# VincentGourbin/ltx-video-swift-mlx

Measured on NVIDIA B200. Metric: dit_steps_per_s, higher is better.
Workload: dtype bf16

## Files before the change

include/ltxcuda.h:

```cpp
#ifndef LTXCUDA_H_
#define LTXCUDA_H_

#include <stddef.h>
#include <stdint.h>

#ifdef __cplusplus
extern "C" {
#endif
#if defined(__GNUC__)
#pragma GCC visibility push(default)
#endif

#define LTX_OK 0
#define LTX_ERR_INVALID_CONFIGURATION 1
#define LTX_ERR_INVALID_ARGUMENT 2
#define LTX_ERR_CUDA 3
#define LTX_ERR_WEIGHTS 4
#define LTX_ERR_UNSUPPORTED 5

typedef enum { LTX_F32 = 0, LTX_BF16 = 1, LTX_F16 = 2 } ltx_dtype;

typedef struct ltx_ctx ltx_ctx;

typedef struct {
  int32_t num_layers;
  int32_t num_heads;
  int32_t head_dim;
  int32_t in_channels;
  int32_t out_channels;
  int32_t caption_channels;
  int32_t ffn_mult;
  float rope_theta;
  int32_t max_pos[3];
  float timestep_scale_multiplier;
  float norm_eps;
  int32_t vae_latent_channels;
  int32_t vae_base_channels;
  int32_t vae_blocks_per_stage;
  int32_t vae_patch_size;
  int32_t vae_encoder_base_channels;
  int32_t upscaler_mid_channels;
  int32_t upscaler_blocks;
  int32_t audio_num_heads;
  int32_t audio_head_dim;
  int32_t audio_in_channels;
  int32_t audio_max_pos;
} ltx_config;

void ltx_config_default(ltx_config* cfg);
const char* ltx_version(void);

int ltx_ctx_create(const ltx_config* cfg, int device, ltx_ctx** out);
int ltx_ctx_destroy(ltx_ctx* ctx);
const char* ltx_last_error(const ltx_ctx* ctx);
int ltx_sync(ltx_ctx* ctx);

int ltx_load_tensor(ltx_ctx* ctx, const char* key, const void* host_data, ltx_dtype dtype, const int64_t* shape, int ndim);
int ltx_load_safetensors(ltx_ctx* ctx, const char* path, int which, int* n_loaded);
int ltx_map_weight_key(int which, const char* file_key, char* out, size_t cap);
int ltx_fuse_lora(ltx_ctx* ctx, const char* key, const void* down, const void* up, ltx_dtype dtype, int rank, float scale);
int ltx_set_precision(ltx_ctx* ctx, int bits);
int ltx_set_quant_storage(ltx_ctx* ctx, int materialise);
int ltx_init_random_weights(ltx_ctx* ctx, int which, uint64_t seed);
int ltx_finalize_weights(ltx_ctx* ctx, int quant_bits, int group_size);

#define LTX_MAX_FLAG_BLOCKS 64
typedef struct {
  int32_t n_stg_blocks;
  int32_t stg_blocks[LTX_MAX_FLAG_BLOCKS];
  int32_t skip_self_attn;
  int32_t skip_ff;
  int32_t n_cas_blocks;
  int32_t cas_blocks[LTX_MAX_FLAG_BLOCKS];
  float cross_attn_scale;
  uint64_t context_key;
} ltx_dit_flags;

int ltx_dit_forward(ltx_ctx* ctx, const void* latent, ltx_dtype latent_dtype, const void* context, ltx_dtype context_dtype,
                    const float* timesteps, int ts_per_token, const int32_t* mask, int B, int N, int S, int F, int H,
                    int W, const ltx_dit_flags* flags, float* out_velocity);
int ltx_dit_forward_dev(ltx_ctx* ctx, const void* latent, ltx_dtype latent_dtype, const void* context,
                        ltx_dtype context_dtype, const float* timesteps, int ts_per_token, const int32_t* mask, int B, int N,
                        int S, int F, int H, int W, const ltx_dit_flags* flags, float* out_velocity);
int ltx_av_forward(ltx_ctx* ctx, const void* video_latent, ltx_dtype video_dtype, const void* audio_latent, ltx_dtype audio_dtype,
                   const void* video_context, const void* audio_context, ltx_dtype context_dtype, float video_sigma,
                   float audio_sigma, const int32_t* video_mask, const int32_t* audio_mask, int N, int Ta, int S, int F, int H,
                   int W, uint64_t context_key, float* out_video, float* out_audio);
int ltx_av_forward_dev(ltx_ctx* ctx, const void* video_latent, ltx_dtype video_dtype, const void* audio_latent,
                       ltx_dtype audio_dtype, const void* video_context, const void* audio_context, ltx_dtype context_dtype,
                       const float* video_sigma, const float* audio_sigma, const int32_t* video_mask, const int32_t* audio_mask,
                       int N, int Ta, int S, int F, int H, int W, uint64_t context_key, float* out_video, float* out_audio);
int ltx_av_forward_tokens(ltx_ctx* ctx, const void* video_latent, ltx_dtype video_dtype, const void* audio_latent,
                          ltx_dtype audio_dtype, const void* video_context, const void* audio_context, ltx_dtype context_dtype,
                          const float* video_sigmas, float audio_sigma, const int32_t* video_mask, const int32_t* audio_mask, int N,
                          int Ta, int S, int F, int H, int W, uint64_t context_key, float* out_video, float* out_audio);
int ltx_av_forward_tokens_dev(ltx_ctx* ctx, const void* video_latent, ltx_dtype video_dtype, const void* audio_latent,
                              ltx_dtype audio_dtype, const void* video_context, const void* audio_context, ltx_dtype context_dtype,
                              const float* video_sigmas, const float* audio_sigma, const int32_t* video_mask,
                              const int32_t* audio_mask, int N, int Ta, int S, int F, int H, int W, uint64_t context_key,
                              float* out_video, float* out_audio);
int ltx_av_forward_batch(ltx_ctx* ctx, const void* video_latent, ltx_dtype video_dtype, const void* audio_latent,
                         ltx_dtype audio_dtype, const void* video_context, const void* audio_context, ltx_dtype context_dtype,
                         const float* video_sigmas, int video_ts_per_token, const float* audio_sigmas, const int32_t* video_mask,
                         const int32_t* audio_mask, int B, int N, int Ta, int S, int F, int H, int W, uint64_t context_key,
                         float* out_video, float* out_audio);
int ltx_av_forward_batch_dev(ltx_ctx* ctx, const void* video_latent, ltx_dtype video_dtype, const void* audio_latent,
                             ltx_dtype audio_dtype, const void* video_context, const void* audio_context, ltx_dtype context_dtype,
                             const float* video_sigmas, int video_ts_per_token, const float* audio_sigmas,
                             const int32_t* video_mask, const int32_t* audio_mask, int B, int N, int Ta, int S, int F, int H, int W,
                             uint64_t context_key, float* out_video, float* out_audio);
int ltx_dit_clear_caches(ltx_ctx* ctx);

int ltx_guided_euler_step(ltx_ctx* ctx, float* latent, const float* v_cond, const float* v_uncond, const float* v_stg,
                          float* v_prev, int use_prev, size_t n, float cfg_scale, float rescale_phi, float stg_scale,
                          float ge_gamma, float sigma, float sigma_next);
int ltx_guided_euler_step_dev(ltx_ctx* ctx, float* latent, const float* v_cond, const float* v_uncond, const float* v_stg,
                              float* v_prev, int use_prev, size_t n, float cfg_scale, float rescale_phi, float stg_scale,
                              float ge_gamma, float sigma, float sigma_next);

typedef struct {
  float sigma, sigma_next;
  float cfg_scale;
  float rescale_phi;
  float stg_scale;
  float ge_gamma;
  int32_t n_stg_blocks;
  int32_t stg_blocks[LTX_MAX_FLAG_BLOCKS];
  int32_t step_index;
  int32_t i2v_frame0_conditioned;
  int32_t disable_stg_prefix_sharing;
  int32_t disable_batched_cfg;
} ltx_step_params;
int ltx_denoise_begin(ltx_ctx* ctx, const float* noise, int F, int H, int W, float sigma0, const void* context,
                      ltx_dtype context_dtype, const int32_t* mask, const void* neg_context, const int32_t* neg_mask, int S);
int ltx_denoise_step(ltx_ctx* ctx, const ltx_step_params* p);
int ltx_denoise_get_latent(ltx_ctx* ctx, float* latent_out);
int ltx_denoise_latent_dev(ltx_ctx* ctx, float** latent_dev);

int ltx_av_denoise_begin(ltx_ctx* ctx, const float* video_noise, const float* audio_noise, int F, int H, int W, int Ta,
                         float sigma0, const void* video_context, const void* audio_context, ltx_dtype context_dtype,
                         const int32_t* mask, const void* neg_video_context, const void* neg_audio_context,
                         const int32_t* neg_mask, int S);
int ltx_av_denoise_step(ltx_ctx* ctx, const ltx_step_params* p);
int ltx_av_denoise_get_latents(ltx_ctx* ctx, float* video_latent_out, float* audio_latent_out);

int ltx_vae_decode(ltx_ctx* ctx, const float* latent, int Fp, int Hp, int Wp, float timestep, const float* decode_noise,
                   int causal, float* out_frames);
int ltx_vae_decode_dev(ltx_ctx* ctx, const float* latent, int Fp, int Hp, int Wp, float timestep,
                       const float* decode_noise, int causal, float* out_frames);
int ltx_vae_tiled_frames(int Fp, int tile_size, int tile_overlap);
int ltx_vae_decode_tiled(ltx_ctx* ctx, const float* latent, int Fp, int Hp, int Wp, float timestep, const float* decode_noise,
                         int causal, int tile_size, int tile_overlap, float* out_frames, int* out_num_frames);
int ltx_vae_decode_tiled_dev(ltx_ctx* ctx, const float* latent, int Fp, int Hp, int Wp, float timestep,
                             const float* decode_noise, int causal, int tile_size, int tile_overlap, float* out_frames,
                             int* out_num_frames);

int ltx_vae_encode(ltx_ctx* ctx, const float* pixels, int T, int H, int W, int normalize, float* latent_out);
int ltx_vae_encode_dev(ltx_ctx* ctx, const float* pixels, int T, int H, int W, int normalize, float* latent_out);

int ltx_upscale_latent(ltx_ctx* ctx, const float* latent, int F, int H, int W, float* out);
int ltx_upscale_latent_dev(ltx_ctx* ctx, const float* latent, int F, int H, int W, float* out);

int ltx_adain_filter(ltx_ctx* ctx, float* latent, size_t n_per_channel, const float* reference, size_t n_ref_per_channel,
                     int channels, float factor);
int ltx_adain_filter_dev(ltx_ctx* ctx, float* latent, size_t n_per_channel, const float* reference, size_t n_ref_per_channel,
                         int channels, float factor);

int ltx_denoise_begin_from_latent(ltx_ctx* ctx, const float* latent, const float* noise, float noise_scale,
                                  const float* frame0_latent, int F, int H, int W, const void* context, ltx_dtype context_dtype,
                                  const int32_t* mask, const void* neg_context, const int32_t* neg_mask, int S);
int ltx_denoise_upscale_stage(ltx_ctx* ctx, const float* noise, float noise_scale, float adain_factor);
int ltx_denoise_set_frame0(ltx_ctx* ctx, const float* frame0_latent);

int ltx_dist_get_unique_id(void* id_out_128);
int ltx_dist_init(ltx_ctx* ctx, const void* unique_id_128, int rank, int world_size, int sp_size, int pass_groups);
int ltx_dist_info(const ltx_ctx* ctx, int* rank, int* world_size, int* sp_size, int* pass_groups);
int ltx_dist_p2p_active(const ltx_ctx* ctx);
int ltx_dist_init_local(ltx_ctx** contexts, int n, int sp_size, int pass_groups);
int ltx_dist_shutdown(ltx_ctx* ctx);

int ltx_host_alloc(void** ptr, size_t bytes);
int ltx_host_free(void* ptr);

uint64_t ltx_launch_count(const ltx_ctx* ctx);
int ltx_get_stream(ltx_ctx* ctx, void** stream);
int ltx_set_profiling(ltx_ctx* ctx, int enabled);
int ltx_set_graphs(ltx_ctx* ctx, int enabled);
int ltx_graph_stats(const ltx_ctx* ctx, uint64_t* captures, uint64_t* replays);
int ltx_get_profile(ltx_ctx* ctx, double* ms, double* flops, double* bytes, uint64_t* counts, int n_classes);

int ltx_op_gemm(ltx_ctx* ctx, const void* A, const void* B, const float* bias, void* C, int M, int N, int K, int mode,
                int force_bn);
int ltx_op_gemm_blocked(ltx_ctx* ctx, const void* A, const void* B, const float* bias, void* plain_out, void* blocks_out, int M, int N,
                        int K, int col_from, int col_block, int64_t block_stride, int force_bn);
int ltx_op_gemm_resid(ltx_ctx* ctx, const void* A, const void* B, const float* bias, float* x, const float* gate_a,
                      const float* gate_b, void* shadow, int M, int N, int K, float scale);
int ltx_op_gemm_skinny(ltx_ctx* ctx, const void* A, const void* B, const float* bias, void* out, float* x, const float* gate_a,
                       const float* gate_b, int rows_per_gate, int M, int N, int K, int mode, int items, int64_t vt_item_ld);
int ltx_op_quantize(ltx_ctx* ctx, const void* w_bf16, int N, int K, int bits, void* q_out, float* scales_out, float* biases_out);
int ltx_op_dequantize(ltx_ctx* ctx, const void* q, const float* scales, const float* biases, int N, int K, int bits, void* w_bf16);
int ltx_op_gemm_q(ltx_ctx* ctx, const void* A, const void* q, const float* scales, const float* biases, int bits,
                  const float* bias, void* C, int M, int N, int K, int mode, int force_bn);
int ltx_op_quantize_fp8(ltx_ctx* ctx, const void* x_bf16, int M, int K, int64_t ld, void* codes, float* scales);
int ltx_op_gemm_fp8(ltx_ctx* ctx, const void* Aq, const float* sa, const void* Bq, const float* sb, const float* bias, void* C, int M,
                    int N, int K, int mode, int force_bn);
int ltx_op_gemm_fp8_ex(ltx_ctx* ctx, const void* Aq, const float* sa, const void* Bq, const float* sb, const float* bias, void* C,
                       void* Ct, int tsplit_col, int64_t ldt, float* x, const float* gate_a, const float* gate_b, void* shadow,
                       int M, int N, int K, int force_bn);
int ltx_op_attention(ltx_ctx* ctx, const void* Q, const void* K, const void* Vt, int64_t ldvb, const float* key_bias, void* O,
                     int B, int H, int Nq, int Nk, float scale);
int ltx_op_attention_hd(ltx_ctx* ctx, const void* Q, const void* K, const void* Vt, int64_t ldvb, const float* key_bias, void* O,
                        int B, int H, int head_dim, int Nq, int Nk, float scale);
int ltx_op_attention_blocks(ltx_ctx* ctx, const void* Q, const void* K, const void* Vt, int64_t ldvb, int H, int Nq, int Nk,
                            float scale, void* const* o_blocks, int n_blocks, int rows_per_block);
int ltx_op_rmsnorm_mod(ltx_ctx* ctx, const float* x, void* out_bf16, int M, int D, const float* tbl_shift,
                       const float* tbl_scale, const float* ada_shift, const float* ada_scale, float eps, int layernorm);
int ltx_op_qknorm_rope(ltx_ctx* ctx, void* x_bf16, int M, int D, const float* w, const float* cos_tab, const float* sin_tab,
                       int rows_per_rope, float eps);
int ltx_conv3d_plan(int T, int H, int W, int Cin, int Cout, int mode, int ntaps, int sm_count, int32_t* plan7);
int ltx_op_conv3d(ltx_ctx* ctx, const float* x, const void* w_bf16_27_O_I, const float* bias, float* out, int T, int H,
                  int W, int Cin, int Cout, int causal);
int ltx_op_vae_prep(ltx_ctx* ctx, const float* x, void* out_pad_bf16, int T, int H, int W, int C, int mode, const float* a,
                    const float* b, int pad);
int ltx_op_vae_halo_fill(ltx_ctx* ctx, void* vol_bf16, int T, int H, int W, int C, int pad);
int ltx_op_conv3d_epi(ltx_ctx* ctx, const void* x_pad_bf16, const void* w_bf16, const float* bias, int T, int H, int W, int Cin,
                      int Cout, int ntaps, int mode, float* out, const float* resid, int t_shift, int no_clip, void* next_pad_bf16,
                      const float* next_scale, const float* next_shift, int next_tshift);

#if defined(__GNUC__)
#pragma GCC visibility pop
#endif
#ifdef __cplusplus
}
#endif
#endif
```

ltx-video-swift-mlx_b200/_lib.py:

```python
from __future__ import annotations

import ctypes as C
import os

_HERE = os.path.dirname(os.path.abspath(__file__))
LIB_PATH = os.path.join(_HERE, "libltxcuda.so")

LTX_F32, LTX_BF16, LTX_F16 = 0, 1, 2
LTX_MAX_FLAG_BLOCKS = 64


class LtxConfig(C.Structure):
    _fields_ = [
        ("num_layers", C.c_int32), ("num_heads", C.c_int32), ("head_dim", C.c_int32), ("in_channels", C.c_int32),
        ("out_channels", C.c_int32), ("caption_channels", C.c_int32), ("ffn_mult", C.c_int32), ("rope_theta", C.c_float),
        ("max_pos", C.c_int32 * 3), ("timestep_scale_multiplier", C.c_float), ("norm_eps", C.c_float),
        ("vae_latent_channels", C.c_int32), ("vae_base_channels", C.c_int32), ("vae_blocks_per_stage", C.c_int32),
        ("vae_patch_size", C.c_int32), ("vae_encoder_base_channels", C.c_int32), ("upscaler_mid_channels", C.c_int32),
        ("upscaler_blocks", C.c_int32), ("audio_num_heads", C.c_int32), ("audio_head_dim", C.c_int32),
        ("audio_in_channels", C.c_int32), ("audio_max_pos", C.c_int32),
    ]


class LtxDitFlags(C.Structure):
    _fields_ = [
        ("n_stg_blocks", C.c_int32), ("stg_blocks", C.c_int32 * LTX_MAX_FLAG_BLOCKS), ("skip_self_attn", C.c_int32),
        ("skip_ff", C.c_int32), ("n_cas_blocks", C.c_int32), ("cas_blocks", C.c_int32 * LTX_MAX_FLAG_BLOCKS),
        ("cross_attn_scale", C.c_float), ("context_key", C.c_uint64),
    ]


class LtxStepParams(C.Structure):
    _fields_ = [
        ("sigma", C.c_float), ("sigma_next", C.c_float), ("cfg_scale", C.c_float), ("rescale_phi", C.c_float),
        ("stg_scale", C.c_float), ("ge_gamma", C.c_float), ("n_stg_blocks", C.c_int32),
        ("stg_blocks", C.c_int32 * LTX_MAX_FLAG_BLOCKS), ("step_index", C.c_int32),
        ("i2v_frame0_conditioned", C.c_int32), ("disable_stg_prefix_sharing", C.c_int32), ("disable_batched_cfg", C.c_int32),
    ]


_P, _I, _F, _U64, _SZ, _I64 = C.c_void_p, C.c_int, C.c_float, C.c_uint64, C.c_size_t, C.c_int64
SIGNATURES = {
    "ltx_config_default": (None, [C.POINTER(LtxConfig)]),
    "ltx_version": (C.c_char_p, []),
    "ltx_ctx_create": (_I, [C.POINTER(LtxConfig), _I, C.POINTER(_P)]),
    "ltx_ctx_destroy": (_I, [_P]),
    "ltx_last_error": (C.c_char_p, [_P]),
    "ltx_sync": (_I, [_P]),
    "ltx_load_tensor": (_I, [_P, C.c_char_p, _P, _I, C.POINTER(_I64), _I]),
    "ltx_load_safetensors": (_I, [_P, C.c_char_p, _I, C.POINTER(_I)]),
    "ltx_map_weight_key": (_I, [_I, C.c_char_p, C.c_char_p, _SZ]),
    "ltx_fuse_lora": (_I, [_P, C.c_char_p, _P, _P, _I, _I, _F]),
    "ltx_set_precision": (_I, [_P, _I]),
    "ltx_set_quant_storage": (_I, [_P, _I]),
    "ltx_init_random_weights": (_I, [_P, _I, _U64]),
    "ltx_finalize_weights": (_I, [_P, _I, _I]),
    "ltx_dit_forward": (_I, [_P, _P, _I, _P, _I, _P, _I, _P, _I, _I, _I, _I, _I, _I, C.POINTER(LtxDitFlags), _P]),
    "ltx_dit_forward_dev": (_I, [_P, _P, _I, _P, _I, _P, _I, _P, _I, _I, _I, _I, _I, _I, C.POINTER(LtxDitFlags), _P]),
    "ltx_av_forward": (_I, [_P, _P, _I, _P, _I, _P, _P, _I, _F, _F, _P, _P, _I, _I, _I, _I, _I, _I, _U64, _P, _P]),
    "ltx_av_forward_dev": (_I, [_P, _P, _I, _P, _I, _P, _P, _I, _P, _P, _P, _P, _I, _I, _I, _I, _I, _I, _U64, _P, _P]),
    "ltx_av_forward_tokens": (_I, [_P, _P, _I, _P, _I, _P, _P, _I, _P, _F, _P, _P, _I, _I, _I, _I, _I, _I, _U64, _P, _P]),
    "ltx_av_forward_tokens_dev": (_I, [_P, _P, _I, _P, _I, _P, _P, _I, _P, _P, _P, _P, _I, _I, _I, _I, _I, _I, _U64, _P, _P]),
    "ltx_av_forward_batch": (_I, [_P, _P, _I, _P, _I, _P, _P, _I, _P, _I, _P, _P, _P, _I, _I, _I, _I, _I, _I, _I, _U64, _P, _P]),
    "ltx_av_forward_batch_dev": (_I, [_P, _P, _I, _P, _I, _P, _P, _I, _P, _I, _P, _P, _P, _I, _I, _I, _I, _I, _I, _I, _U64, _P, _P]),
    "ltx_dit_clear_caches": (_I, [_P]),
    "ltx_guided_euler_step": (_I, [_P, _P, _P, _P, _P, _P, _I, _SZ, _F, _F, _F, _F, _F, _F]),
    "ltx_guided_euler_step_dev": (_I, [_P, _P, _P, _P, _P, _P, _I, _SZ, _F, _F, _F, _F, _F, _F]),
    "ltx_denoise_begin": (_I, [_P, _P, _I, _I, _I, _F, _P, _I, _P, _P, _P, _I]),
    "ltx_denoise_step": (_I, [_P, C.POINTER(LtxStepParams)]),
    "ltx_denoise_get_latent": (_I, [_P, _P]),
    "ltx_denoise_latent_dev": (_I, [_P, C.POINTER(_P)]),
    "ltx_av_denoise_begin": (_I, [_P, _P, _P, _I, _I, _I, _I, _F, _P, _P, _I, _P, _P, _P, _P, _I]),
    "ltx_av_denoise_step": (_I, [_P, C.POINTER(LtxStepParams)]),
    "ltx_av_denoise_get_latents": (_I, [_P, _P, _P]),
    "ltx_vae_decode": (_I, [_P, _P, _I, _I, _I, _F, _P, _I, _P]),
    "ltx_vae_decode_dev": (_I, [_P, _P, _I, _I, _I, _F, _P, _I, _P]),
    "ltx_vae_tiled_frames": (_I, [_I, _I, _I]),
    "ltx_vae_decode_tiled": (_I, [_P, _P, _I, _I, _I, _F, _P, _I, _I, _I, _P, _P]),
    "ltx_vae_decode_tiled_dev": (_I, [_P, _P, _I, _I, _I, _F, _P, _I, _I, _I, _P, _P]),
    "ltx_vae_encode": (_I, [_P, _P, _I, _I, _I, _I, _P]),
    "ltx_vae_encode_dev": (_I, [_P, _P, _I, _I, _I, _I, _P]),
    "ltx_upscale_latent": (_I, [_P, _P, _I, _I, _I, _P]),
    "ltx_upscale_latent_dev": (_I, [_P, _P, _I, _I, _I, _P]),
    "ltx_adain_filter": (_I, [_P, _P, _SZ, _P, _SZ, _I, _F]),
    "ltx_adain_filter_dev": (_I, [_P, _P, _SZ, _P, _SZ, _I, _F]),
    "ltx_denoise_begin_from_latent": (_I, [_P, _P, _P, _F, _P, _I, _I, _I, _P, _I, _P, _P, _P, _I]),
    "ltx_denoise_upscale_stage": (_I, [_P, _P, _F, _F]),
    "ltx_denoise_set_frame0": (_I, [_P, _P]),
    "ltx_dist_get_unique_id": (_I, [_P]),
    "ltx_dist_init": (_I, [_P, _P, _I, _I, _I, _I]),
    "ltx_dist_init_local": (_I, [_P, _I, _I, _I]),
    "ltx_dist_shutdown": (_I, [_P]),
    "ltx_dist_p2p_active": (_I, [_P]),
    "ltx_dist_info": (_I, [_P, C.POINTER(_I), C.POINTER(_I), C.POINTER(_I), C.POINTER(_I)]),
    "ltx_host_alloc": (_I, [C.POINTER(_P), _SZ]),
    "ltx_host_free": (_I, [_P]),
    "ltx_launch_count": (_U64, [_P]),
    "ltx_get_stream": (_I, [_P, C.POINTER(_P)]),
    "ltx_set_profiling": (_I, [_P, _I]),
    "ltx_set_graphs": (_I, [_P, _I]),
    "ltx_graph_stats": (_I, [_P, _P, _P]),
    "ltx_get_profile": (_I, [_P, _P, _P, _P, _P, _I]),
    "ltx_op_gemm": (_I, [_P, _P, _P, _P, _P, _I, _I, _I, _I, _I]),
    "ltx_op_gemm_blocked": (_I, [_P, _P, _P, _P, _P, _P, _I, _I, _I, _I, _I, C.c_int64, _I]),
    "ltx_op_gemm_resid": (_I, [_P, _P, _P, _P, _P, _P, _P, _P, _I, _I, _I, _F]),
    "ltx_op_gemm_skinny": (_I, [_P, _P, _P, _P, _P, _P, _P, _P, _I, _I, _I, _I, _I, _I, C.c_int64]),
    "ltx_op_quantize": (_I, [_P, _P, _I, _I, _I, _P, _P, _P]),
    "ltx_op_dequantize": (_I, [_P, _P, _P, _P, _I, _I, _I, _P]),
    "ltx_op_gemm_q": (_I, [_P, _P, _P, _P, _P, _I, _P, _P, _I, _I, _I, _I, _I]),
    "ltx_op_quantize_fp8": (_I, [_P, _P, _I, _I, _I64, _P, _P]),
    "ltx_op_gemm_fp8": (_I, [_P, _P, _P, _P, _P, _P, _P, _I, _I, _I, _I, _I]),
    "ltx_op_gemm_fp8_ex": (_I, [_P, _P, _P, _P, _P, _P, _P, _P, _I, _I64, _P, _P, _P, _P, _I, _I, _I, _I]),
    "ltx_op_attention": (_I, [_P, _P, _P, _P, _I64, _P, _P, _I, _I, _I, _I, _F]),
    "ltx_op_attention_hd": (_I, [_P, _P, _P, _P, _I64, _P, _P, _I, _I, _I, _I, _I, _F]),
    "ltx_op_attention_blocks": (_I, [_P, _P, _P, _P, _I64, _I, _I, _I, _F, C.POINTER(_P), _I, _I]),
    "ltx_op_rmsnorm_mod": (_I, [_P, _P, _P, _I, _I, _P, _P, _P, _P, _F, _I]),
    "ltx_op_qknorm_rope": (_I, [_P, _P, _I, _I, _P, _P, _P, _I, _F]),
    "ltx_op_conv3d": (_I, [_P, _P, _P, _P, _P, _I, _I, _I, _I, _I, _I]),
    "ltx_conv3d_plan": (_I, [_I, _I, _I, _I, _I, _I, _I, _I, C.POINTER(C.c_int32)]),
    "ltx_op_vae_prep": (_I, [_P, _P, _P, _I, _I, _I, _I, _I, _P, _P, _I]),
    "ltx_op_vae_halo_fill": (_I, [_P, _P, _I, _I, _I, _I, _I]),
    "ltx_op_conv3d_epi": (_I, [_P, _P, _P, _P, _I, _I, _I, _I, _I, _I, _I, _P, _P, _I, _I, _P, _P, _P, _I]),
}

_lib = None


def load() -> C.CDLL:
    global _lib
    if _lib is not None:
        return _lib
    if not os.path.exists(LIB_PATH):
        raise RuntimeError(
            f"{LIB_PATH} is missing: build it with `bash ltx-video-swift-mlx_b200/csrc/build.sh` "
            "(there is no CPU / PyTorch fallback for the product path)")
    lib = C.CDLL(LIB_PATH)
    for name, (res, args) in SIGNATURES.items():
        fn = getattr(lib, name)
        fn.restype = res
        fn.argtypes = args
    _lib = lib
    return lib


class LtxError(RuntimeError):

    def __init__(self, code: int, message: str):
        super().__init__(f"[ltxcuda error {code}] {message}")
        self.code = code
```

ltx-video-swift-mlx_b200/csrc/api.cu:

```cuda
#include <cstring>

#include "ctx.h"

using namespace ltx;

namespace {

thread_local std::string g_create_error;

template <typename Fn>
int guarded(ltx_ctx* c, Fn&& fn) {
  if (!c) return LTX_ERR_INVALID_ARGUMENT;
  try {
    LTX_CUDA(cudaSetDevice(c->device));
    fn();
    return LTX_OK;
  } catch (const LtxError& e) {
    c->last_error = e.what();
    return e.code;
  } catch (const std::exception& e) {
    c->last_error = e.what();
    return LTX_ERR_CUDA;
  }
}
// ... 915 lines not shown
    h2d(c, c->s_latent, video_noise, n * 4);
    h2d(c, c->s_alat, audio_noise, na * 4);
    {
      ProfScope ps(c, PROF_OTHER, 0.0, 8.0 * (n + na), 2);
      launch_scale_f32(c->s_latent.as<float>(), sigma0, static_cast<int64_t>(n), c->stream);
      launch_scale_f32(c->s_alat.as<float>(), sigma0, static_cast<int64_t>(na), c->stream);
    }
    const size_t cbytes = static_cast<size_t>(S) * g.caption_channels * dsize(context_dtype);
    h2d(c, c->s_ctx_pos, video_context, cbytes);
    h2d(c, c->s_actx_pos, audio_context, cbytes);
    c->s_has_mask_pos = mask != nullptr;
    if (mask) h2d(c, c->s_mask_pos, mask, static_cast<size_t>(S) * 4);
    c->s_has_neg = neg_video_context != nullptr;
    if (c->s_has_neg) {
      h2d(c, c->s_ctx_neg, neg_video_context, cbytes);
      h2d(c, c->s_actx_neg, neg_audio_context, cbytes);
      c->s_has_mask_neg = neg_mask != nullptr;
      if (neg_mask) h2d(c, c->s_mask_neg, neg_mask, static_cast<size_t>(S) * 4);
      c->s_ctx_pair.reserve(2 * cbytes);
      c->s_actx_pair.reserve(2 * cbytes);
      LTX_CUDA(cudaMemcpyAsync(c->s_ctx_pair.ptr, c->s_ctx_pos.ptr, cbytes, cudaMemcpyDeviceToDevice, c->stream));
      LTX_CUDA(cudaMemcpyAsync(c->s_ctx_pair.as<uint8_t>() + cbytes, c->s_ctx_neg.ptr, cbytes, cudaMemcpyDeviceToDevice, c->stream));
      LTX_CUDA(cudaMemcpyAsync(c->s_actx_pair.ptr, c->s_actx_pos.ptr, cbytes, cudaMemcpyDeviceToDevice, c->stream));
      LTX_CUDA(cudaMemcpyAsync(c->s_actx_pair.as<uint8_t>() + cbytes, c->s_actx_neg.ptr, cbytes, cudaMemcpyDeviceToDevice, c->stream));
      if (mask || neg_mask) {
        std::vector<int32_t> pm(static_cast<size_t>(2) * S, 1);
        if (mask) memcpy(pm.data(), mask, static_cast<size_t>(S) * 4);
        if (neg_mask) memcpy(pm.data() + S, neg_mask, static_cast<size_t>(S) * 4);
        h2d(c, c->s_mask_pair, pm.data(), pm.size() * 4);
        LTX_CUDA(cudaStreamSynchronize(c->stream));
      }
      c->s_tok.reserve(2 * n * 2);
      c->vel.reserve(2 * n * 4);
      c->s_alat_pair.reserve(2 * na * 4);
    }
    c->s_avc.reserve((c->s_has_neg ? 2 : 1) * na * 4);
    c->s_avu.reserve(na * 4);
    c->scratch.reserve(64 * sizeof(double));
    c->s_serial += 2;
    dit_clear_caches(c);
    LTX_CUDA(cudaStreamSynchronize(c->stream));
  });
}

int ltx_av_denoise_step(ltx_ctx* c, const ltx_step_params* p) {
  return guarded(c, [&] {
    av_precision_check(c);
    LTX_CHECK(p != nullptr && c->s_F > 0 && c->s_Ta > 0, LTX_ERR_INVALID_ARGUMENT, "av_denoise_step before av_denoise_begin");
    LTX_CHECK(p->sigma > 0.f, LTX_ERR_INVALID_ARGUMENT, "sigma must be > 0");
    LTX_CHECK(p->stg_scale == 0.f && p->ge_gamma == 0.f, LTX_ERR_UNSUPPORTED,
              "the audio + video loop has no STG / GE terms (Pipeline/LTXPipeline.swift:1300-1404)");
    const ltx_config& g = c->cfg;
    const int C = g.in_channels, F = c->s_F, H = c->s_H, W = c->s_W, S = c->s_S, Ta = c->s_Ta;
    const int T = F * H * W;
    const size_t n = static_cast<size_t>(C) * T, na = static_cast<size_t>(Ta) * c->av.Cin;
    cudaStream_t st = c->stream;
    {
      ProfScope ps(c, PROF_OTHER, 0.0, 6.0 * n);
      launch_patchify(c->s_latent.as<float>(), c->s_tok.as<bf16>(), nullptr, C, T, st);
    }
    const bool use_cfg = p->cfg_scale > 1.0f && c->s_has_neg;
    const bool batched = batched_cfg_env() && use_cfg && c->dist.groups == 1 && !(c->dist.comm_world && c->dist.sp > 1) &&
                         !p->disable_batched_cfg;
    const int nb = batched ? 2 : 1;
    const float sig2[2] = {p->sigma, p->sigma};
    LTX_CUDA(cudaMemcpyAsync(c->s_sigma.ptr, sig2, 8, cudaMemcpyHostToDevice, st));
    const bool i2v = p->i2v_frame0_conditioned != 0;
    const float* ts_dev = c->s_sigma.as<float>();
    if (i2v) {
      c->s_ts.reserve(static_cast<size_t>(nb) * T * 4);
      ProfScope ps(c, PROF_OTHER, 0.0, 4.0 * nb * T);
      launch_fill_token_timesteps(c->s_ts.as<float>(), nb * T, T, H * W, c->s_sigma.as<float>(), st);
      ts_dev = c->s_ts.as<float>();
    }
    const uint64_t key_pos = 0x6000000000000000ull + c->s_serial, key_neg = key_pos + 1;
    const uint64_t key_pair = 0x6800000000000000ull + c->s_serial;
    auto pass = [&](bool neg, float* v_lat, float* a_vel) {
      const int32_t* mk = neg ? (c->s_has_mask_neg ? c->s_mask_neg.as<int32_t>() : nullptr)
                              : (c->s_has_mask_pos ? c->s_mask_pos.as<int32_t>() : nullptr);
      dit_av_forward_dev(c, c->s_tok.ptr, LTX_BF16, c->s_alat.ptr, LTX_F32, neg ? c->s_ctx_neg.ptr : c->s_ctx_pos.ptr,
                         neg ? c->s_actx_neg.ptr : c->s_actx_pos.ptr, c->s_ctx_dtype, ts_dev, i2v ? 1 : 0, c->s_sigma.as<float>(), mk,
                         mk, 1, T, Ta, S, F, H, W, neg ? key_neg : key_pos, c->vel.as<float>(), a_vel);
      ProfScope ps(c, PROF_OTHER, 0.0, 8.0 * n);
      launch_unpatchify(c->vel.as<float>(), v_lat, C, T, st);
    };
    float* avu = c->s_avu.as<float>();
    if (batched) {
      bf16* tok = c->s_tok.as<bf16>();
      float* alat2 = c->s_alat_pair.as<float>();
      LTX_CUDA(cudaMemcpyAsync(tok + n, tok, n * 2, cudaMemcpyDeviceToDevice, st));
      LTX_CUDA(cudaMemcpyAsync(alat2, c->s_alat.ptr, na * 4, cudaMemcpyDeviceToDevice, st));
      LTX_CUDA(cudaMemcpyAsync(alat2 + na, c->s_alat.ptr, na * 4, cudaMemcpyDeviceToDevice, st));
      const int32_t* mk = (c->s_has_mask_pos || c->s_has_mask_neg) ? c->s_mask_pair.as<int32_t>() : nullptr;
      avu = c->s_avc.as<float>() + na;
      dit_av_forward_dev(c, tok, LTX_BF16, alat2, LTX_F32, c->s_ctx_pair.ptr, c->s_actx_pair.ptr, c->s_ctx_dtype, ts_dev, i2v ? 1 : 0,
                         c->s_sigma.as<float>(), mk, mk, 2, T, Ta, S, F, H, W, key_pair, c->vel.as<float>(), c->s_avc.as<float>());
      ProfScope ps(c, PROF_OTHER, 0.0, 16.0 * n, 2);
      launch_unpatchify(c->vel.as<float>(), c->s_vc.as<float>(), C, T, st);
      launch_unpatchify(c->vel.as<float>() + n, c->s_vu.as<float>(), C, T, st);
    } else {
      pass(false, c->s_vc.as<float>(), c->s_avc.as<float>());
      if (use_cfg) pass(true, c->s_vu.as<float>(), avu);
    }
    GuidedEulerArgs a;
    a.latent = c->s_latent.as<float>(); a.v_cond = c->s_vc.as<float>();
    a.v_uncond = use_cfg ? c->s_vu.as<float>() : nullptr;
    a.v_stg = nullptr; a.v_prev = nullptr; a.use_prev = 0;
    a.v_out = nullptr; a.n = n; a.cfg = use_cfg ? p->cfg_scale : 1.0f; a.phi = use_cfg ? p->rescale_phi : 0.0f; a.stg = 0.f;
    a.ge_gamma = 0.f; a.sigma = p->sigma; a.sigma_next = p->sigma_next; a.scratch = c->scratch.as<double>();
    if (i2v) { a.period = static_cast<size_t>(T); a.frozen = static_cast<size_t>(H) * W; }
    ProfScope ps(c, PROF_OTHER, 0.0, 4.0 * n * (3.0 + (use_cfg ? 1.0 : 0.0)) + 4.0 * na * (3.0 + (use_cfg ? 1.0 : 0.0)),
                 ((use_cfg && p->rescale_phi > 0.f) ? 2 : 1) + 1);
    launch_guided_euler(a, st);
    const float dt = static_cast<float>(static_cast<double>(p->sigma_next) - static_cast<double>(p->sigma));
    launch_audio_cfg_euler(c->s_alat.as<float>(), c->s_avc.as<float>(), use_cfg ? avu : nullptr, p->cfg_scale, dt,
                           static_cast<int64_t>(na), st);
  });
}

int ltx_av_denoise_get_latents(ltx_ctx* c, float* video_out, float* audio_out) {
  return guarded(c, [&] {
    LTX_CHECK(c->s_F > 0 && c->s_Ta > 0, LTX_ERR_INVALID_ARGUMENT, "no audio + video denoise session");
    const size_t n = static_cast<size_t>(c->cfg.in_channels) * c->s_F * c->s_H * c->s_W;
    if (video_out) LTX_CUDA(cudaMemcpyAsync(video_out, c->s_latent.ptr, n * 4, cudaMemcpyDeviceToHost, c->stream));
    if (audio_out)
      LTX_CUDA(cudaMemcpyAsync(audio_out, c->s_alat.ptr, static_cast<size_t>(c->s_Ta) * c->av.Cin * 4, cudaMemcpyDeviceToHost,
                               c->stream));
    LTX_CUDA(cudaStreamSynchronize(c->stream));
  });
}

int ltx_vae_decode_dev(ltx_ctx* c, const float* latent, int Fp, int Hp, int Wp, float timestep, const float* decode_noise,
                       int causal, float* out_frames) {
  return guarded(c, [&] { vae_decode_dev(c, latent, Fp, Hp, Wp, timestep, decode_noise, causal, out_frames); });
}

int ltx_vae_decode(ltx_ctx* c, const float* latent, int Fp, int Hp, int Wp, float timestep, const float* decode_noise,
                   int causal, float* out_frames) {
  return guarded(c, [&] {
    LTX_CHECK(latent && out_frames && Fp > 0 && Hp > 0 && Wp > 0, LTX_ERR_INVALID_ARGUMENT, "bad vae_decode arguments");
    const size_t n = static_cast<size_t>(c->cfg.vae_latent_channels) * Fp * Hp * Wp;
    h2d(c, c->v_lat, latent, n * 4);
    const float* nz = nullptr;
    if (timestep >= 0.f) {
      LTX_CHECK(decode_noise != nullptr, LTX_ERR_INVALID_ARGUMENT, "decode_noise is required when timestep >= 0");
      h2d(c, c->v_noise, decode_noise, n * 4);
      nz = c->v_noise.as<float>();
    }
    const size_t fo = static_cast<size_t>(8 * (Fp - 1) + 1) * (32 * Hp) * (32 * Wp) * 3;
    c->v_frames.reserve(fo * 4);
    vae_decode_dev(c, c->v_lat.as<float>(), Fp, Hp, Wp, timestep, nz, causal, c->v_frames.as<float>());
    LTX_CUDA(cudaMemcpyAsync(out_frames, c->v_frames.ptr, fo * 4, cudaMemcpyDeviceToHost, c->stream));
    LTX_CUDA(cudaStreamSynchronize(c->stream));
  });
}

int ltx_vae_tiled_frames(int Fp, int tile_size, int tile_overlap) {
  if (Fp <= 0 || (tile_size > 0 && Fp > tile_size && (tile_overlap < 0 || tile_overlap >= tile_size))) return -1;
  return vae_tiled_frames(Fp, tile_size, tile_overlap);
}

int ltx_vae_decode_tiled_dev(ltx_ctx* c, const float* latent, int Fp, int Hp, int Wp, float timestep, const float* decode_noise,
                             int causal, int tile_size, int tile_overlap, float* out_frames, int* out_num_frames) {
  return guarded(c, [&] {
    const int n = vae_decode_tiled_dev(c, latent, Fp, Hp, Wp, timestep, decode_noise, causal, tile_size, tile_overlap, out_frames);
    if (out_num_frames) *out_num_frames = n;
  });
}

int ltx_vae_decode_tiled(ltx_ctx* c, const float* latent, int Fp, int Hp, int Wp, float timestep, const float* decode_noise,
                         int causal, int tile_size, int tile_overlap, float* out_frames, int* out_num_frames) {
  return guarded(c, [&] {
    LTX_CHECK(latent && out_frames && Fp > 0 && Hp > 0 && Wp > 0, LTX_ERR_INVALID_ARGUMENT, "bad vae_decode arguments");
    const int nf = ltx_vae_tiled_frames(Fp, tile_size, tile_overlap);
    LTX_CHECK(nf > 0, LTX_ERR_INVALID_ARGUMENT, "temporal tile overlap must be in [0, tile size)");
    const size_t n = static_cast<size_t>(c->cfg.vae_latent_channels) * Fp * Hp * Wp;
    h2d(c, c->v_lat, latent, n * 4);
    const float* nz = nullptr;
    if (timestep >= 0.f) {
      LTX_CHECK(decode_noise != nullptr, LTX_ERR_INVALID_ARGUMENT, "decode_noise is required when timestep >= 0");
      h2d(c, c->v_noise, decode_noise, n * 4);
      nz = c->v_noise.as<float>();
    }
    const size_t fe = static_cast<size_t>(32 * Hp) * (32 * Wp) * 3;
    c->v_frames.reserve(static_cast<size_t>(nf) * fe * 4);
    const int got = vae_decode_tiled_dev(c, c->v_lat.as<float>(), Fp, Hp, Wp, timestep, nz, causal, tile_size, tile_overlap,
                                         c->v_frames.as<float>());
    LTX_CHECK(got == nf, LTX_ERR_CUDA, "tiled decode frame count mismatch");
    if (out_num_frames) *out_num_frames = got;
    LTX_CUDA(cudaMemcpyAsync(out_frames, c->v_frames.ptr, static_cast<size_t>(got) * fe * 4, cudaMemcpyDeviceToHost, c->stream));
    LTX_CUDA(cudaStreamSynchronize(c->stream));
  });
}

int ltx_vae_encode_dev(ltx_ctx* c, const float* pixels, int T, int H, int W, int normalize, float* latent_out) {
  return guarded(c, [&] { vae_encode_dev(c, pixels, T, H, W, normalize, latent_out); });
}

int ltx_vae_encode(ltx_ctx* c, const float* pixels, int T, int H, int W, int normalize, float* latent_out) {
  return guarded(c, [&] {
    LTX_CHECK(pixels && latent_out && T >= 1 && H >= 64 && W >= 64 && H % 32 == 0 && W % 32 == 0, LTX_ERR_INVALID_ARGUMENT,
              "bad vae_encode arguments");
    const size_t n_in = static_cast<size_t>(3) * T * H * W;
    const size_t n_out = static_cast<size_t>(c->cfg.vae_latent_channels) * ((T + 7) / 8) * (H / 32) * (W / 32);
    h2d(c, c->u_in, pixels, n_in * 4);
    c->u_out.reserve(n_out * 4);
    vae_encode_dev(c, c->u_in.as<float>(), T, H, W, normalize, c->u_out.as<float>());
    LTX_CUDA(cudaMemcpyAsync(latent_out, c->u_out.ptr, n_out * 4, cudaMemcpyDeviceToHost, c->stream));
    LTX_CUDA(cudaStreamSynchronize(c->stream));
  });
}

int ltx_upscale_latent_dev(ltx_ctx* c, const float* latent, int F, int H, int W, float* out) {
  return guarded(c, [&] { upscale_latent_dev(c, latent, F, H, W, out); });
}

int ltx_upscale_latent(ltx_ctx* c, const float* latent, int F, int H, int W, float* out) {
  return guarded(c, [&] {
    LTX_CHECK(latent && out && F >= 1 && H > 1 && W > 1, LTX_ERR_INVALID_ARGUMENT, "bad upscale_latent arguments");
    const size_t n = static_cast<size_t>(c->cfg.vae_latent_channels) * F * H * W;
    h2d(c, c->u_in, latent, n * 4);
    c->u_out.reserve(4 * n * 4);
    upscale_latent_dev(c, c->u_in.as<float>(), F, H, W, c->u_out.as<float>());
    LTX_CUDA(cudaMemcpyAsync(out, c->u_out.ptr, 4 * n * 4, cudaMemcpyDeviceToHost, c->stream));
    LTX_CUDA(cudaStreamSynchronize(c->stream));
  });
}

int ltx_adain_filter_dev(ltx_ctx* c, float* latent, size_t n_per_channel, const float* reference, size_t n_ref_per_channel,
                         int channels, float factor) {
  return guarded(c, [&] {
    adain_filter_dev(c, latent, static_cast<int64_t>(n_per_channel), reference, static_cast<int64_t>(n_ref_per_channel), channels,
                     factor);
  });
}

int ltx_adain_filter(ltx_ctx* c, float* latent, size_t n_per_channel, const float* reference, size_t n_ref_per_channel, int channels,
                     float factor) {
  return guarded(c, [&] {
    LTX_CHECK(latent && reference && channels > 0, LTX_ERR_INVALID_ARGUMENT, "bad adain arguments");
    h2d(c, c->u_in, latent, n_per_channel * channels * 4);
    h2d(c, c->u_ref, reference, n_ref_per_channel * channels * 4);
    adain_filter_dev(c, c->u_in.as<float>(), static_cast<int64_t>(n_per_channel), c->u_ref.as<float>(),
                     static_cast<int64_t>(n_ref_per_channel), channels, factor);
    LTX_CUDA(cudaMemcpyAsync(latent, c->u_in.ptr, n_per_channel * channels * 4, cudaMemcpyDeviceToHost, c->stream));
    LTX_CUDA(cudaStreamSynchronize(c->stream));
  });
}

int ltx_op_gemm(ltx_ctx* c, const void* A, const void* B, const float* bias, void* C, int M, int N, int K, int mode,
                int force_bn) {
  return guarded(c, [&] {
    GemmEpi e;
    e.mode = mode; e.out = C; e.ldo = N; e.bias = bias;
    LTX_CHECK(mode == EPI_BF16 || mode == EPI_GELU_BF16 || mode == EPI_F32 || mode == EPI_SILU_BF16, LTX_ERR_INVALID_ARGUMENT, "bad mode");
    if (force_bn == -1) {
      LTX_CHECK(gemm_skinny_eligible(K, K, M, N, K, e, 0), LTX_ERR_INVALID_ARGUMENT, "shape not eligible for the skinny GEMM");
      launch_gemm_skinny(reinterpret_cast<const bf16*>(A), K, reinterpret_cast<const bf16*>(B), K, M, N, K, e, c->stream);
    } else if (force_bn == -2 || force_bn == -3) {
      LTX_CHECK(gemm_swapab_eligible(K, K, M, N, K, e), LTX_ERR_INVALID_ARGUMENT, "shape not eligible for the swap-AB GEMM");
      if (force_bn == -2) gemm_attach_workspace(c, e);
      launch_gemm_swapab(reinterpret_cast<const bf16*>(A), K, reinterpret_cast<const bf16*>(B), K, M, N, K, e, c->stream);
    } else {
      launch_gemm(reinterpret_cast<const bf16*>(A), K, reinterpret_cast<const bf16*>(B), K, M, N, K, e, c->stream, force_bn);
    }
    c->launches++;
  });
}

int ltx_op_gemm_blocked(ltx_ctx* c, const void* A, const void* B, const float* bias, void* plain_out, void* blocks_out, int M, int N,
                        int K, int col_from, int col_block, int64_t block_stride, int force_bn) {
  return guarded(c, [&] {
    LTX_CHECK(col_block > 0 && col_from >= 0 && col_from < N && (N - col_from) % col_block == 0 && (N - col_from) / col_block <= LTX_MAX_PEERS,
              LTX_ERR_INVALID_ARGUMENT, "bad column blocking");
    GemmEpi e;
    e.mode = EPI_BF16; e.out = plain_out; e.ldo = col_from > 0 ? col_from : col_block; e.bias = bias;
    e.col_block = col_block; e.col_block_from = col_from; e.blocked_ld = col_block; e.use_col_ptrs = 1;
    for (int j = 0; j < (N - col_from) / col_block; ++j)
      e.col_ptrs.p[j] = reinterpret_cast<bf16*>(blocks_out) + static_cast<int64_t>(j) * block_stride;
    if (force_bn == -2) {
      gemm_attach_workspace(c, e);
      launch_gemm_swapab(reinterpret_cast<const bf16*>(A), K, reinterpret_cast<const bf16*>(B), K, M, N, K, e, c->stream);
    } else {
      launch_gemm(reinterpret_cast<const bf16*>(A), K, reinterpret_cast<const bf16*>(B), K, M, N, K, e, c->stream, force_bn);
    }
    c->launches++;
  });
}

int ltx_op_gemm_resid(ltx_ctx* c, const void* A, const void* B, const float* bias, float* x, const float* gate_a,
                      const float* gate_b, void* shadow, int M, int N, int K, float scale) {
  return guarded(c, [&] {
    GemmEpi e;
    e.mode = EPI_GATE_RESID; e.resid = x; e.ldr = N; e.bias = bias; e.gate_a = gate_a; e.gate_b = gate_b; e.gate_ld = 0;
    e.rows_per_gate = M > 0 ? M : 1; e.shadow = reinterpret_cast<bf16*>(shadow); e.lds = N; e.scale = scale;
    if (M > 32 && M <= 512) gemm_attach_workspace(c, e);
    const char* fb = getenv("LTX_GEMM_FORCE_BN");
    launch_gemm(reinterpret_cast<const bf16*>(A), K, reinterpret_cast<const bf16*>(B), K, M, N, K, e, c->stream, fb ? atoi(fb) : 0, 0, 0,
                32 );
    c->launches++;
  });
}

int ltx_op_gemm_skinny(ltx_ctx* c, const void* A, const void* B, const float* bias, void* out, float* x, const float* gate_a,
                       const float* gate_b, int rows_per_gate, int M, int N, int K, int mode, int items, int64_t vt_item_ld) {
  return guarded(c, [&] {
    LTX_CHECK(A && B && (mode == EPI_GATE_RESID ? x != nullptr : out != nullptr) && (items == 1 || items == 2) &&
                  (vt_item_ld == 0 || (M % items == 0 && vt_item_ld >= M / items)),
              LTX_ERR_INVALID_ARGUMENT, "bad skinny GEMM arguments");
    LTX_CHECK(mode >= EPI_BF16 && mode <= EPI_SILU_BF16 && (vt_item_ld == 0 || mode == EPI_BF16), LTX_ERR_INVALID_ARGUMENT, "bad mode");
    GemmEpi e;
    e.mode = mode; e.bias = bias;
    if (mode == EPI_GATE_RESID) {
      e.resid = x; e.ldr = N; e.gate_a = gate_a; e.gate_b = gate_b; e.gate_ld = N;
      e.rows_per_gate = rows_per_gate > 0 ? rows_per_gate : M;
    } else if (vt_item_ld > 0) {
      e.out = out; e.ldo = items * vt_item_ld; e.transpose_out = 1;
      if (items > 1) { e.t_item_rows = M / items; e.t_item_ld = vt_item_ld; }
    } else {
      e.out = out; e.ldo = N;
    }
    LTX_CHECK(gemm_skinny_eligible(K, K, M, N, K, e, 0, 32 * items), LTX_ERR_INVALID_ARGUMENT, "shape not eligible for the skinny GEMM");
    launch_gemm(reinterpret_cast<const bf16*>(A), K, reinterpret_cast<const bf16*>(B), K, M, N, K, e, c->stream, 0, 0, 0, 32 * items);
    c->launches++;
  });
}

int ltx_op_quantize(ltx_ctx* c, const void* w_bf16, int N, int K, int bits, void* q_out, float* scales_out, float* biases_out) {
  return guarded(c, [&] {
    launch_quantize(reinterpret_cast<const bf16*>(w_bf16), N, K, bits, reinterpret_cast<uint8_t*>(q_out), scales_out, biases_out,
                    c->stream);
    c->launches++;
  });
}

int ltx_op_dequantize(ltx_ctx* c, const void* q, const float* scales, const float* biases, int N, int K, int bits, void* w_bf16) {
  return guarded(c, [&] {
    QuantW W;
    W.q = reinterpret_cast<const uint8_t*>(q); W.scales = scales; W.biases = biases; W.bits = bits; W.n = N; W.k = K;
    launch_dequantize(W, reinterpret_cast<bf16*>(w_bf16), c->stream);
    c->launches++;
  });
}

int ltx_op_gemm_q(ltx_ctx* c, const void* A, const void* q, const float* scales, const float* biases, int bits, const float* bias,
                  void* C, int M, int N, int K, int mode, int force_bn) {
  return guarded(c, [&] {
    LTX_CHECK(mode == EPI_BF16 || mode == EPI_GELU_BF16 || mode == EPI_F32, LTX_ERR_INVALID_ARGUMENT, "bad mode");
    QuantW W;
    W.q = reinterpret_cast<const uint8_t*>(q); W.scales = scales; W.biases = biases; W.bits = bits; W.n = N; W.k = K;
    GemmEpi e;
    e.mode = mode; e.out = C; e.ldo = N; e.bias = bias;
    launch_gemm_q(reinterpret_cast<const bf16*>(A), K, W, M, N, K, e, c->stream, force_bn);
    c->launches++;
  });
}

int ltx_op_quantize_fp8(ltx_ctx* c, const void* x_bf16, int M, int K, int64_t ld, void* codes, float* scales) {
  return guarded(c, [&] {
    LTX_CHECK(x_bf16 && codes && scales, LTX_ERR_INVALID_ARGUMENT, "null tensor");
    launch_quantize_rows_fp8(reinterpret_cast<const bf16*>(x_bf16), ld, M, K, reinterpret_cast<uint8_t*>(codes), scales, c->stream);
    c->launches++;
  });
}

int ltx_op_gemm_fp8(ltx_ctx* c, const void* Aq, const float* sa, const void* Bq, const float* sb, const float* bias, void* C, int M,
                    int N, int K, int mode, int force_bn) {
  return guarded(c, [&] {
    LTX_CHECK(Aq && sa && Bq && sb && C, LTX_ERR_INVALID_ARGUMENT, "null tensor");
    LTX_CHECK(mode == EPI_BF16 || mode == EPI_GELU_BF16 || mode == EPI_F32 || mode == EPI_SILU_BF16, LTX_ERR_INVALID_ARGUMENT, "bad mode");
    GemmEpi e;
    e.mode = mode; e.out = C; e.ldo = N; e.bias = bias;
    launch_gemm_fp8(reinterpret_cast<const uint8_t*>(Aq), K, sa, reinterpret_cast<const uint8_t*>(Bq), K, sb, M, N, K, e, c->stream,
                    force_bn);
    c->launches++;
  });
}

int ltx_op_gemm_fp8_ex(ltx_ctx* c, const void* Aq, const float* sa, const void* Bq, const float* sb, const float* bias, void* C,
                       void* Ct, int tsplit_col, int64_t ldt, float* x, const float* gate_a, const float* gate_b, void* shadow,
                       int M, int N, int K, int force_bn) {
  return guarded(c, [&] {
    LTX_CHECK(Aq && sa && Bq && sb && (x != nullptr) != (C != nullptr), LTX_ERR_INVALID_ARGUMENT,
              "bad FP8 GEMM arguments: one of C (bf16, with optional V^T split) or x (gate * residual)");
    GemmEpi e;
    e.bias = bias;
    if (x) {
      e.mode = EPI_GATE_RESID; e.resid = x; e.ldr = N; e.gate_a = gate_a; e.gate_b = gate_b; e.gate_ld = 0;
      e.rows_per_gate = M; e.shadow = reinterpret_cast<bf16*>(shadow); e.lds = N;
    } else {
      e.mode = EPI_BF16; e.out = C; e.ldo = tsplit_col > 0 ? tsplit_col : N;
      if (tsplit_col > 0) { e.tsplit_col = tsplit_col; e.out_t = reinterpret_cast<bf16*>(Ct); e.ldt = ldt; }
    }
    launch_gemm_fp8(reinterpret_cast<const uint8_t*>(Aq), K, sa, reinterpret_cast<const uint8_t*>(Bq), K, sb, M, N, K, e, c->stream,
                    force_bn);
    c->launches++;
  });
}

int ltx_op_attention(ltx_ctx* c, const void* Q, const void* K, const void* Vt, int64_t ldvb, const float* key_bias, void* O,
                     int B, int H, int Nq, int Nk, float scale) {
  return guarded(c, [&] {
    const int D = H * 128;
    launch_attention(reinterpret_cast<const bf16*>(Q), D, reinterpret_cast<const bf16*>(K), D,
                     reinterpret_cast<const bf16*>(Vt), ldvb, key_bias, reinterpret_cast<bf16*>(O), D, B, H, Nq, Nk, D, scale,
                     c->stream);
    c->launches++;
  });
}

int ltx_op_attention_hd(ltx_ctx* c, const void* Q, const void* K, const void* Vt, int64_t ldvb, const float* key_bias, void* O,
                        int B, int H, int head_dim, int Nq, int Nk, float scale) {
  return guarded(c, [&] {
    LTX_CHECK(head_dim == 128 || head_dim == 64, LTX_ERR_UNSUPPORTED, "head_dim must be 128 or 64");
    const int D = H * head_dim;
    launch_attention(reinterpret_cast<const bf16*>(Q), D, reinterpret_cast<const bf16*>(K), D,
                     reinterpret_cast<const bf16*>(Vt), ldvb, key_bias, reinterpret_cast<bf16*>(O), D, B, H, Nq, Nk, D, scale,
                     c->stream);
    c->launches++;
  });
}

int ltx_op_attention_blocks(ltx_ctx* c, const void* Q, const void* K, const void* Vt, int64_t ldvb, int H, int Nq, int Nk,
                            float scale, void* const* o_blocks, int n_blocks, int rows_per_block) {
  return guarded(c, [&] {
    LTX_CHECK(o_blocks && n_blocks >= 1 && n_blocks <= LTX_MAX_PEERS && rows_per_block > 0 && n_blocks * rows_per_block >= Nq,
              LTX_ERR_INVALID_ARGUMENT, "bad output blocks");
    const int D = H * 128;
    PeerTable t = {};
    for (int i = 0; i < n_blocks; ++i) t.p[i] = o_blocks[i];
    launch_attention(reinterpret_cast<const bf16*>(Q), D, reinterpret_cast<const bf16*>(K), D, reinterpret_cast<const bf16*>(Vt), ldvb,
                     nullptr, reinterpret_cast<bf16*>(o_blocks[0]), D, 1, H, Nq, Nk, D, scale, c->stream, &t, rows_per_block);
    c->launches++;
  });
}

int ltx_op_rmsnorm_mod(ltx_ctx* c, const float* x, void* out_bf16, int M, int D, const float* tbl_shift,
                       const float* tbl_scale, const float* ada_shift, const float* ada_scale, float eps, int layernorm) {
  return guarded(c, [&] {
    launch_rmsnorm_mod(x, reinterpret_cast<bf16*>(out_bf16), M, D, tbl_shift, tbl_scale, ada_shift, ada_scale, 0, M, eps,
                       layernorm, c->stream);
    c->launches++;
  });
}

int ltx_op_qknorm_rope(ltx_ctx* c, void* x_bf16, int M, int D, const float* w, const float* cos_tab, const float* sin_tab,
                       int rows_per_rope, float eps) {
  return guarded(c, [&] {
    launch_qknorm_rope(reinterpret_cast<bf16*>(x_bf16), D, M, D, w, cos_tab, sin_tab, rows_per_rope, eps, c->stream);
    c->launches++;
  });
}

int ltx_conv3d_plan(int T, int H, int W, int Cin, int Cout, int mode, int ntaps, int sm_count, int32_t* plan7) {
  if (plan7 == nullptr || T <= 0 || H <= 1 || W <= 1 || Cin <= 0 || Cout <= 0 || (ntaps != 27 && ntaps != 9) || sm_count <= 0 || mode < 0 ||
      mode > 4)
    return LTX_ERR_INVALID_ARGUMENT;
  const ConvPlan p = conv3d_plan(T, H, W, Cin, Cout, mode, ntaps, true, sm_count, conv3d_pair_default(), conv3d_slab_default());
  plan7[0] = p.bn; plan7[1] = p.pair; plan7[2] = p.slab; plan7[3] = p.bt; plan7[4] = p.bh; plan7[5] = p.bw; plan7[6] = p.ksplit;
  return LTX_OK;
}

int ltx_op_conv3d(ltx_ctx* c, const float* x, const void* w, const float* bias, float* out, int T, int H, int W, int Cin,
                  int Cout, int causal) {
  return guarded(c, [&] {
    c->v_pad.reserve(static_cast<size_t>(T + 2) * (H + 2) * (W + 2) * Cin * 2);
    launch_vae_prep(x, c->v_pad.as<bf16>(), T, H, W, Cin, 0, nullptr, nullptr, causal, c->stream);
    ConvEpi e;
    e.mode = 0; e.out = out; e.bias = bias; e.resid = nullptr; e.Cin = Cin;
    float* scratch = nullptr;
    const size_t slab3 = static_cast<size_t>(3) * T * H * W * Cout * 4;
    if (conv3d_wants_tap_split(H, W, Cin, Cout)) {
      c->v_split.reserve(slab3);
      scratch = c->v_split.as<float>();
    }
    launch_conv3d(c->v_pad.as<bf16>(), reinterpret_cast<const bf16*>(w), T, H, W, Cin, Cout, e, c->stream, 27, scratch, scratch ? slab3 : 0);
    c->launches += 2;
  });
}

int ltx_op_vae_prep(ltx_ctx* c, const float* x, void* out_pad, int T, int H, int W, int C, int mode, const float* a, const float* b,
                    int pad) {
  return guarded(c, [&] {
    launch_vae_prep(x, reinterpret_cast<bf16*>(out_pad), T, H, W, C, mode, a, b, pad, c->stream);
    c->launches++;
  });
}

int ltx_op_vae_halo_fill(ltx_ctx* c, void* vol, int T, int H, int W, int C, int pad) {
  return guarded(c, [&] {
    launch_vae_halo_fill(reinterpret_cast<bf16*>(vol), T, H, W, C, pad, c->stream);
    c->launches++;
  });
}

int ltx_op_conv3d_epi(ltx_ctx* c, const void* x_pad, const void* w, const float* bias, int T, int H, int W, int Cin, int Cout,
                      int ntaps, int mode, float* out, const float* resid, int t_shift, int no_clip, void* next_pad,
                      const float* next_scale, const float* next_shift, int next_tshift) {
  return guarded(c, [&] {
    ConvEpi e;
    e.mode = mode; e.out = out; e.bias = bias; e.resid = resid; e.Cin = Cin; e.t_shift = t_shift; e.no_clip = no_clip;
    e.next_pad = reinterpret_cast<bf16*>(next_pad); e.next_scale = next_scale; e.next_shift = next_shift; e.next_tshift = next_tshift;
    float* scratch = nullptr;
    const size_t slab3 = static_cast<size_t>(3) * T * H * W * Cout * 4;
    if (mode == 0 && ntaps == 27 && conv3d_wants_tap_split(H, W, Cin, Cout)) {
      c->v_split.reserve(slab3);
      scratch = c->v_split.as<float>();
    }
    launch_conv3d(reinterpret_cast<const bf16*>(x_pad), reinterpret_cast<const bf16*>(w), T, H, W, Cin, Cout, e, c->stream, ntaps,
                  scratch, scratch ? slab3 : 0);
    c->launches++;
  });
}

}
```

ltx-video-swift-mlx_b200/csrc/ctx.h:

```cpp
#pragma once
#include <atomic>
#include <map>
#include <string>
#include <vector>

#include "../../include/ltxcuda.h"
#include "ltx_internal.h"

namespace ltx {

struct DevTensor {
  void* ptr = nullptr;
  int dtype = LTX_F32;
  std::vector<int64_t> shape;
  int64_t numel() const {
    int64_t n = 1;
    for (auto d : shape) n *= d;
    return n;
  }
};

inline std::atomic<uint64_t>& devbuf_generation() {
  static std::atomic<uint64_t> g{1};
  return g;
}

struct DevBuf {
  void* ptr = nullptr;
  size_t bytes = 0;
  void reserve(size_t n) {
    if (n <= bytes) return;
    devbuf_generation().fetch_add(1, std::memory_order_relaxed);
    if (ptr) LTX_CUDA(cudaFree(ptr));
    ptr = nullptr;
    bytes = 0;
    LTX_CUDA(cudaMalloc(&ptr, n));
    bytes = n;
  }
  void release() {
    if (ptr) { devbuf_generation().fetch_add(1, std::memory_order_relaxed); cudaFree(ptr); }
    ptr = nullptr;
    bytes = 0;
  }
  template <typename T>
  T* as() const { return reinterpret_cast<T*>(ptr); }
};

enum LinearFormat : int {
  LW_BF16 = 0,
  LW_AFFINE = 1,
  LW_E4M3 = 2,
};
struct LinearW {
  int fmt = LW_BF16;
  int n = 0, k = 0;
  const bf16* w = nullptr;
  QuantW q;
};

struct AdaLnW {
  const bf16 *w1 = nullptr, *w2 = nullptr, *wl = nullptr;
  const float *b1 = nullptr, *b2 = nullptr, *bl = nullptr;
  int dim = 0, n = 0;
};

struct AttnWeights {
  LinearW wq, wk, wv, wo;
  const float *bq = nullptr, *bk = nullptr, *bv = nullptr, *bo = nullptr;
  const float *q_norm = nullptr, *k_norm = nullptr;
};

struct BlockWeights {
  const float* sst = nullptr;
  AttnWeights a1, a2;
  LinearW w_in, w_out;
  const float *b_in = nullptr, *b_out = nullptr;
};

struct TextCache {
  uint64_t key = 0;
  uint64_t fingerprint = 0;
  int B = 0, S = 0;
  int64_t ldv = 0;
  DevBuf k;
  DevBuf vt;
  DevBuf bias;
  bool has_bias = false;
};

struct TextProjW {
  LinearW w_c1, w_c2;
  const float *b_c1 = nullptr, *b_c2 = nullptr;
  int D = 0;
  const void* user = nullptr;
  const AttnWeights& (*layer)(const void* user, int i) = nullptr;
};

struct ConvW {
  const bf16* w = nullptr;
  const float* b = nullptr;
  int cin = 0, cout = 0;
  int taps = 27;
};
struct VaeResBlock {
  ConvW c1, c2;
  const float* sst = nullptr;
};
struct VaeTimeEmb {
  const bf16 *w1 = nullptr, *w2 = nullptr;
  const float *b1 = nullptr, *b2 = nullptr;
  int out = 0;
};
struct VaeWeights {
  bool ready = false;
  bool has_time = false;
  float ts_mult = 1000.0f;
  VaeTimeEmb stage_te[4], last_te;
  const float *mean = nullptr, *std = nullptr;
  ConvW conv_in, conv_out;
  std::vector<std::vector<VaeResBlock>> stages;
  std::vector<ConvW> ups;
  const float* last_sst = nullptr;
};

struct AvBlockW {
  const float *norm1 = nullptr, *norm2 = nullptr, *norm3 = nullptr, *a2v_norm = nullptr;
  const float *anorm1 = nullptr, *anorm2 = nullptr, *anorm3 = nullptr, *v2a_norm = nullptr;
  AttnWeights aa1, aa2, a2v, v2a;
  LinearW w_in, w_out;
  const float *b_in = nullptr, *b_out = nullptr;
  const float *asst = nullptr;
  const float *sst_ca_v = nullptr;
  const float *sst_ca_a = nullptr;
};
struct AvWeights {
  bool ready = false;
  int Da = 0, Ha = 0, hd = 0, Cin = 0;
  LinearW w_patch, w_c1, w_c2, w_out;
  const float *b_patch = nullptr, *b_c1 = nullptr, *b_c2 = nullptr, *b_out = nullptr, *sst_out = nullptr;
  AdaLnW ada_a, cv_ss, cv_g, ca_ss, ca_g;
  std::vector<AvBlockW> blocks;
  TextCache text[2];
  int text_rr = 0;
  DevBuf ws;
  DevBuf a_cos, a_sin, xv_cos, xv_sin;
  int rope_ta = 0, rope_f = 0, rope_hw = 0;
};

struct EncResBlock { ConvW c1, c2; };
struct EncStage {
  std::vector<EncResBlock> res;
  ConvW down;
  int cout = 0;
};
struct EncWeights {
  bool ready = false;
  int base = 0;
  ConvW conv_in, conv_out;
  EncStage stage[4];
  std::vector<EncResBlock> mid;
};
struct GnW { const float *w = nullptr, *b = nullptr; };
struct UpsBlock { ConvW c1, c2; GnW n1, n2; };
struct UpsWeights {
  bool ready = false;
  int mid = 0, cin = 0;
  ConvW initial, up2d, final_conv;
  GnW initial_norm;
  std::vector<UpsBlock> pre, post;
};

}

namespace ltx {
struct DistState {
  bool p2p_tried = false, p2p = false;
  void* p2p_local = nullptr;
  size_t p2p_bytes = 0;
  void* p2p_peer[8] = {};
  bool p2p_ipc[8] = {};
  void* p2p_pool = nullptr;
  void* comm_world = nullptr;
  void* comm_sp = nullptr;
  bool sp_is_world = true;
  int rank = 0, world = 1, sp = 1, groups = 1, group = 0, sp_rank = 0;
};
struct StepGraph {
  int state = 0;
  cudaGraphExec_t exec = nullptr;
  uint64_t launches = 0;
  uint64_t generation = 0;
  uint64_t last_use = 0;
};
enum ProfClass { PROF_GEMM = 0, PROF_ATTN = 1, PROF_ROW = 2, PROF_CONV = 3, PROF_PREP = 4, PROF_OTHER = 5, PROF_COMM = 6, PROF_NCLASS = 8 };
struct ProfRec {
  cudaEvent_t a, b;
  int cls;
  double flops, bytes;
};
}

struct ltx_ctx {
  ltx_config cfg;
  ltx::DistState dist;
  bool prof_on = false;
  std::vector<ltx::ProfRec> prof_recs;
  std::vector<cudaEvent_t> prof_pool;

  std::map<std::string, ltx::StepGraph> graphs;
  uint64_t graph_clock = 0, graph_replays = 0, graph_captures = 0;
  int graphs_enabled = 1;

  int device = 0;
  cudaStream_t stream = nullptr;
  mutable std::string last_error;
  uint64_t launches = 0;

  std::map<std::string, ltx::DevTensor> tensors;
  int quant_bits = 16;
  int quant_materialise = 0;
  ltx::DevBuf q_panel;
  ltx::DevBuf gemm_ws;
  std::vector<void*> owned;
  bool dit_ready = false;
  std::vector<ltx::BlockWeights> blocks;
  ltx::LinearW w_patch, w_c1, w_c2, w_out;
  const float *b_patch = nullptr, *b_c1 = nullptr, *b_c2 = nullptr, *b_out = nullptr, *sst_out = nullptr;
  ltx::AdaLnW adaln;
  ltx::VaeWeights vae;
  ltx::AvWeights av;
  ltx::EncWeights enc;
  ltx::UpsWeights ups;

  ltx::DevBuf lat_in, ctx_in, ts_in, mask_in;
  ltx::DevBuf api_lat, api_ctx;
  ltx::DevBuf x, xb, h, qk, vt, att, q2, ffh, vel;
  ltx::DevBuf se, t1, emb, ada;
  ltx::DevBuf c1, c2;
  ltx::DevBuf rope_cos, rope_sin;
  int rope_f = 0, rope_h = 0, rope_w = 0;
  ltx::TextCache text[2];
  int text_rr = 0;
  ltx::DevBuf scratch;
  ltx::DevBuf sp_send, sp_recv, sp_vt, sp_vel;
  ltx::DevBuf snap_x;
  int snap_rows = 0;

  int precision = 16;
  ltx::DevBuf fp8_act;
  ltx::DevBuf f_asplit, f_wsplit, f_h, f_q, f_k, f_v, f_att, f_ffh, f_ctx, f_c1, f_c2, f_tk, f_tv, f_lat, f_bias;

  ltx::DevBuf s_latent, s_tok, s_vc, s_vu, s_vs, s_vprev, s_ctx_pos, s_ctx_neg, s_mask_pos, s_mask_neg, s_sigma, s_ts;
  ltx::DevBuf s_ctx_pair, s_mask_pair;
  int s_F = 0, s_H = 0, s_W = 0, s_S = 0;
  bool s_has_neg = false, s_has_mask_pos = false, s_has_mask_neg = false;
  int s_ctx_dtype = LTX_BF16;
  uint64_t s_serial = 0;
  ltx::DevBuf s_alat, s_avc, s_avu, s_actx_pos, s_actx_neg;
  ltx::DevBuf s_alat_pair, s_actx_pair;
  int s_Ta = 0;

  ltx::DevBuf v_a, v_b, v_h, v_pad, v_lat, v_noise, v_frames, v_mix, v_te, v_split, v_pad2;
  ltx::DevBuf v_tile_lat, v_tile_noise, v_tile_frames;
  int vae_no_clip = 0;
  ltx::DevBuf av_in[8];
  ltx::DevBuf u_part, u_ab, u_stats, u_in, u_out, u_ref;
};

namespace ltx {
void gemm_attach_workspace(ltx_ctx* c, GemmEpi& e);
struct ProfScope {
  ltx_ctx* c;
  ProfRec r;
  bool on;
  ProfScope(ltx_ctx* ctx, int cls, double flops, double bytes, int launches = 1) : c(ctx), on(ctx->prof_on) {
    c->launches += launches;
    if (!on) return;
    auto get = [&]() {
      cudaEvent_t e;
      if (!c->prof_pool.empty()) { e = c->prof_pool.back(); c->prof_pool.pop_back(); }
      else LTX_CUDA(cudaEventCreate(&e));
      return e;
    };
    r.a = get(); r.b = get(); r.cls = cls; r.flops = flops; r.bytes = bytes;
    LTX_CUDA(cudaEventRecord(r.a, c->stream));
  }
  ~ProfScope() {
    if (!on) return;
    cudaEventRecord(r.b, c->stream);
    c->prof_recs.push_back(r);
  }
};
void graphs_clear(ltx_ctx* c);
struct LinearOpts {
  int allow_skinny = 0;
  bool split_k = false;
  int tile_n = 0;
  int a_kblock = 0;
  int64_t a_kblock_stride = 0;
};
void linear(ltx_ctx* c, const bf16* A, int64_t lda, const LinearW& W, int M, int N, int K, const GemmEpi& e, const LinearOpts& o);
void linear_vt(ltx_ctx* c, const bf16* A, int rows, int items, const LinearW& W, const float* bias, bf16* out, int64_t ld_out,
               int64_t item_ld, bf16* tmp, const LinearOpts& o);
void attention(ltx_ctx* c, const bf16* Q, int64_t ldq, const bf16* K, int64_t ldk, const bf16* Vt, int64_t ldv, const float* bias,
               bf16* O, int64_t ldo, int B, int H, int Nq, int Nk, int D, const PeerTable* o_blocks = nullptr,
               int rows_per_block = 0);
void adaln_single(ltx_ctx* c, const AdaLnW& a, float* se, float* t1, float* emb, float* lin, int B, const float* sigma = nullptr,
                  float mult = 0.f);
void adaln_single_rows(ltx_ctx* c, const AdaLnW& a, const bf16* se_bf, int R, bf16* t1_bf, float* emb, float* lin, int64_t ld_lin,
                       const LinearOpts& o);
const bf16* wbf(ltx_ctx* c, const std::string& k, int64_t r, int64_t cc);
const float* wf(ltx_ctx* c, const std::string& k, int64_t n);
LinearW wlin(ltx_ctx* c, const std::string& k, int64_t n, int64_t kk);
AdaLnW adaln_w(ltx_ctx* c, const std::string& p, int64_t dim, int n);
void dit_finalize(ltx_ctx* c);
void dit_quantize(ltx_ctx* c, int bits);
void dit_convert_fp8(ltx_ctx* c);
void dit_forward_dev(ltx_ctx* c, const void* latent, int latent_dtype, const void* context, int context_dtype,
                     const float* timesteps_dev, int ts_per_token, const int32_t* mask_dev, int B, int N, int S, int F,
                     int H, int W, const ltx_dit_flags* flags, float* out_velocity_dev, int snapshot_block = -1,
                     int resume_block = -1);
void dit_clear_caches(ltx_ctx* c);
TextCache& dit_prepare_text(ltx_ctx* c, TextCache* slots, int* rr, const TextProjW& src, const void* context, int context_dtype,
                            const int32_t* mask_dev, int B, int S, uint64_t key);
void dit_build_rope(ltx_ctx* c, int F, int H, int W);
void dit_av_finalize(ltx_ctx* c);
void dit_av_forward_dev(ltx_ctx* c, const void* v_latent, int v_dtype, const void* a_latent, int a_dtype, const void* v_context,
                        const void* a_context, int ctx_dtype, const float* v_ts_dev, int v_ts_per_token, const float* a_ts_dev,
                        const int32_t* v_mask_dev, const int32_t* a_mask_dev, int B, int N, int Ta, int S, int F, int H, int W, uint64_t context_key,
                        float* out_v_dev, float* out_a_dev);
void dit_finalize_f32(ltx_ctx* c);
void dit_forward_f32(ltx_ctx* c, const void* latent, int latent_dtype, const void* context, int context_dtype,
                     const float* timesteps_dev, int ts_per_token, const int32_t* mask_dev, int B, int N, int S, int F, int H,
                     int W, const ltx_dit_flags* flags, float* out_velocity_dev);
void vae_finalize(ltx_ctx* c);
int vae_tiled_frames(int Fp, int tile_size, int overlap);
int vae_decode_tiled_dev(ltx_ctx* c, const float* latent_dev, int Fp, int Hp, int Wp, float timestep, const float* noise_dev,
                         int causal, int tile_size, int tile_overlap, float* frames_dev);
void vae_decode_dev(ltx_ctx* c, const float* latent_dev, int Fp, int Hp, int Wp, float timestep, const float* noise_dev,
                    int causal, float* frames_dev);
ConvW vae_pack_conv_keys(ltx_ctx* c, const std::string& wkey, const std::string& bkey, int64_t cout, int64_t cin,
                         int64_t cout_use, int taps);
const float* vae_vec(ltx_ctx* c, const std::string& key, int64_t n);
void vae_conv(ltx_ctx* c, const float* x, int prep_mode, const float* a, const float* b, const ConvW& w, int T, int H, int W,
              int pad, int epi_mode, float* out, const float* resid, int n_active = 1, int t_shift = 0);
void vae_encoder_finalize(ltx_ctx* c);
void vae_encode_dev(ltx_ctx* c, const float* pixels_dev, int T, int H, int W, int normalize, float* latent_dev);
void upscaler_finalize(ltx_ctx* c);
void upscale_latent_dev(ltx_ctx* c, const float* latent_dev, int F, int H, int W, float* out_dev);
void adain_filter_dev(ltx_ctx* c, float* latent_dev, int64_t n_per_channel, const float* ref_dev, int64_t n_ref_per_channel,
                      int C, float factor);
void renoise_dev(ltx_ctx* c, float* latent_dev, const float* noise_dev, int64_t n, float noise_scale);
void dist_get_unique_id(void* out128);
void dist_init(ltx_ctx* c, const void* unique_id, int rank, int world_size, int sp_size, int pass_groups);
void dist_init_local(ltx_ctx** contexts, int n, int sp_size, int pass_groups);
void dist_destroy(ltx_ctx* c);
void dist_broadcast(ltx_ctx* c, void* buf, size_t bytes, int root_world_rank);
void dist_allgather_sp(ltx_ctx* c, const void* send, void* recv, size_t bytes_per_rank);
void dist_all_to_all_sp(ltx_ctx* c, const void* const* send, void* const* recv, int n_tensors, size_t bytes_per_peer);
bool dist_p2p_ensure(ltx_ctx* c, size_t bytes);
void dist_p2p_barrier(ltx_ctx* c, int kind);
void dist_halo_exchange(ltx_ctx* c, const void* send_prev, void* recv_prev, const void* send_next, void* recv_next,
                        size_t bytes, int n_active);
std::string map_transformer_key(const std::string& file_key, bool include_audio = false);
std::string map_vae_key(const std::string& file_key);
std::string map_vae_encoder_key(const std::string& file_key);
std::string map_upscaler_key(const std::string& file_key);
int load_safetensors(ltx_ctx* c, const char* path, int which);
const DevTensor& get_tensor(ltx_ctx* c, const std::string& key);
void load_tensor_host(ltx_ctx* c, const std::string& key, const void* host, int dtype, const int64_t* shape, int ndim);
void init_random_weights(ltx_ctx* c, int which, uint64_t seed);
void fuse_lora(ltx_ctx* c, const std::string& key, const void* down_host, const void* up_host, int dtype, int rank, float scale);
std::string map_lora_key(const std::string& lora_key);
}
```

ltx-video-swift-mlx_b200/csrc/dit.cu:

```cuda
#include <algorithm>
#include <cmath>

#include "ctx.h"

namespace ltx {

namespace {

double gemm_bytes(int M, int N, int K) {
  return 2.0 * (static_cast<double>(M) * K + static_cast<double>(N) * K + static_cast<double>(M) * N);
}
void gemm_bf16(ltx_ctx* c, const bf16* A, int64_t lda, const bf16* B, int64_t ldb, int M, int N, int K, const GemmEpi& e,
               const LinearOpts& o) {
  ProfScope ps(c, PROF_GEMM, 2.0 * M * N * K, gemm_bytes(M, N, K));
  GemmEpi ew = e;
  if (o.split_k && M <= 512) gemm_attach_workspace(c, ew);
  const int force_bn = o.tile_n == 0 ? 0 : M > 128 ? 1000 + o.tile_n : o.tile_n;
  launch_gemm(A, lda, B, ldb, M, N, K, ew, c->stream, force_bn, o.a_kblock, o.a_kblock_stride, o.allow_skinny);
}

}

void linear(ltx_ctx* c, const bf16* A, int64_t lda, const LinearW& W, int M, int N, int K, const GemmEpi& e, const LinearOpts& o) {
  LTX_CHECK(W.k == K && N >= 1 && N <= W.n, LTX_ERR_INVALID_ARGUMENT, "Linear: weight shape mismatch");
  if (W.fmt == LW_BF16) {
    gemm_bf16(c, A, lda, W.w, K, M, N, K, e, o);
  } else if (W.fmt == LW_AFFINE) {
    ProfScope ps(c, PROF_GEMM, 2.0 * M * N * K, gemm_bytes(M, N, K), gemm_q_uses_panel(W.q, M) ? 2 : 1);
    launch_gemm_q(A, lda, W.q, M, N, K, e, c->stream, 0, o.a_kblock, o.a_kblock_stride);
  } else {
    LTX_CHECK(o.a_kblock == 0, LTX_ERR_UNSUPPORTED, "FP8 GEMM: no K-blocked A operand");
    const size_t code_bytes = (static_cast<size_t>(M) * K + 15) / 16 * 16;
    c->fp8_act.reserve(code_bytes + static_cast<size_t>(M) * 4);
    uint8_t* q = c->fp8_act.as<uint8_t>();
    float* s = reinterpret_cast<float*>(q + code_bytes);
    {
      ProfScope ps(c, PROF_ROW, 0.0, 3.0 * M * K + 4.0 * M);
      launch_quantize_rows_fp8(A, lda, M, K, q, s, c->stream);
    }
    ProfScope ps(c, PROF_GEMM, 2.0 * M * N * K, static_cast<double>(M) * K + static_cast<double>(N) * K + 2.0 * M * N);
    launch_gemm_fp8(q, K, s, W.q.q, W.q.k, W.q.scales, M, N, K, e, c->stream, o.tile_n);
  }
}

void linear_vt(ltx_ctx* c, const bf16* A, int rows, int items, const LinearW& W, const float* bias, bf16* out, int64_t ld_out,
               int64_t item_ld, bf16* tmp, const LinearOpts& o) {
  const int N = W.n, K = W.k;
  GemmEpi e;
  e.mode = EPI_BF16; e.bias = bias;
  if (W.fmt != LW_BF16) {
    e.out = tmp; e.ldo = N;
    linear(c, A, K, W, items * rows, N, K, e, o);
    ProfScope ps(c, PROF_OTHER, 0.0, 4.0 * items * rows * N, items);
    for (int i = 0; i < items; ++i)
      launch_transpose_bf16(tmp + static_cast<int64_t>(i) * rows * N, N, rows, N, out + i * item_ld, ld_out, c->stream);
    return;
  }
  e.out = out; e.ldo = ld_out;
  if (items > 1) { e.t_item_rows = rows; e.t_item_ld = item_ld; }
  if (gemm_skinny_eligible(K, K, items * rows, N, K, e, 0, o.allow_skinny)) {
    e.transpose_out = 1;
    linear(c, A, K, W, items * rows, N, K, e, o);
    return;
  }
  e.t_item_rows = 0;
  e.bias_per_row = 1;
  if (items == 1 || rows == item_ld) {
    gemm_bf16(c, W.w, K, A, K, N, items * rows, K, e, o);
    return;
  }
  for (int i = 0; i < items; ++i) {
    e.out = out + i * item_ld;
    gemm_bf16(c, W.w, K, A + static_cast<int64_t>(i) * rows * K, K, N, rows, K, e, o);
  }
}

void attention(ltx_ctx* c, const bf16* Q, int64_t ldq, const bf16* K, int64_t ldk, const bf16* Vt, int64_t ldv, const float* bias,
               bf16* O, int64_t ldo, int B, int H, int Nq, int Nk, int D, const PeerTable* o_blocks, int rows_per_block) {
  const int hd = D / H;
  ProfScope ps(c, PROF_ATTN, 4.0 * B * H * static_cast<double>(Nq) * Nk * hd, 2.0 * B * (2.0 * Nq + 2.0 * Nk) * D);
  launch_attention(Q, ldq, K, ldk, Vt, ldv, bias, O, ldo, B, H, Nq, Nk, D, 1.0f / sqrtf(static_cast<float>(hd)), c->stream, o_blocks,
                   rows_per_block);
}

void adaln_single(ltx_ctx* c, const AdaLnW& a, float* se, float* t1, float* emb, float* lin, int B, const float* sigma, float mult) {
  ProfScope ps(c, PROF_OTHER, 2.0 * B * a.dim * (256.0 + (1.0 + a.n) * a.dim), 2.0 * a.dim * (256.0 + (1.0 + a.n) * a.dim),
               sigma ? 4 : 3);
  if (sigma) launch_sincos_embed(sigma, mult, se, B, 256, c->stream);
  launch_gemv(a.w1, a.b1, se, t1, B, a.dim, 256, 0, c->stream);
  launch_gemv(a.w2, a.b2, t1, emb, B, a.dim, a.dim, 1, c->stream);
  launch_gemv(a.wl, a.bl, emb, lin, B, a.n * a.dim, a.dim, 1, c->stream);
}

void adaln_single_rows(ltx_ctx* c, const AdaLnW& a, const bf16* se_bf, int R, bf16* t1_bf, float* emb, float* lin, int64_t ld_lin,
                       const LinearOpts& o) {
  GemmEpi e1;
  e1.mode = EPI_SILU_BF16; e1.out = t1_bf; e1.ldo = a.dim; e1.bias = a.b1;
  gemm_bf16(c, se_bf, 256, a.w1, 256, R, a.dim, 256, e1, o);
  GemmEpi e2;
  e2.mode = EPI_F32; e2.out = emb; e2.ldo = a.dim; e2.bias = a.b2;
  gemm_bf16(c, t1_bf, a.dim, a.w2, a.dim, R, a.dim, a.dim, e2, o);
  {
    ProfScope ps(c, PROF_OTHER, 0.0, 6.0 * R * a.dim);
    launch_silu_cast(emb, t1_bf, static_cast<int64_t>(R) * a.dim, c->stream);
  }
  GemmEpi e3;
  e3.mode = EPI_F32; e3.out = lin; e3.ldo = ld_lin; e3.bias = a.bl;
  gemm_bf16(c, t1_bf, a.dim, a.wl, a.dim, R, a.n * a.dim, a.dim, e3, o);
}

const bf16* wbf(ltx_ctx* c, const std::string& k, int64_t r, int64_t cc) {
  const DevTensor& t = get_tensor(c, k);
  LTX_CHECK(t.dtype == LTX_BF16 && t.shape.size() == 2 && t.shape[0] == r && t.shape[1] == cc, LTX_ERR_WEIGHTS,
            "bad shape for '" + k + "'");
  return reinterpret_cast<const bf16*>(t.ptr);
}
const float* wf(ltx_ctx* c, const std::string& k, int64_t n) {
  const DevTensor& t = get_tensor(c, k);
  LTX_CHECK(t.dtype == LTX_F32 && t.numel() == n, LTX_ERR_WEIGHTS, "bad shape for '" + k + "'");
  return reinterpret_cast<const float*>(t.ptr);
}
LinearW wlin(ltx_ctx* c, const std::string& k, int64_t n, int64_t kk) {
  LinearW w;
  w.n = static_cast<int>(n); w.k = static_cast<int>(kk); w.w = wbf(c, k, n, kk);
  return w;
}
AdaLnW adaln_w(ltx_ctx* c, const std::string& p, int64_t dim, int n) {
  AdaLnW a;
  a.w1 = wbf(c, p + ".emb.linear_1.weight", dim, 256); a.b1 = wf(c, p + ".emb.linear_1.bias", dim);
  a.w2 = wbf(c, p + ".emb.linear_2.weight", dim, dim); a.b2 = wf(c, p + ".emb.linear_2.bias", dim);
  a.wl = wbf(c, p + ".linear.weight", n * dim, dim); a.bl = wf(c, p + ".linear.bias", n * dim);
  a.dim = static_cast<int>(dim); a.n = n;
  return a;
}

namespace {

void norm_mod(ltx_ctx* c, const float* x, bf16* out, int M, int D, const float* ts, const float* tsc, const float* as,
              const float* asc, int64_t ada_ld, int rows_per_mod, float eps, int ln) {
  ProfScope ps(c, PROF_ROW, 0.0, static_cast<double>(M) * D * 6.0);
  launch_rmsnorm_mod(x, out, M, D, ts, tsc, as, asc, ada_ld, rows_per_mod, eps, ln, c->stream);
}
void qknorm(ltx_ctx* c, bf16* x, int64_t ld, int M, int D, const float* w, const float* cs, const float* sn, int rpr,
            float eps, const float* w_second = nullptr, const QkOut* blocked = nullptr) {
  const int segs = w_second ? 2 : 1;
  ProfScope ps(c, PROF_ROW, 0.0, segs * static_cast<double>(M) * D * (4.0 + (cs ? 4.0 : 0.0)), (D == 4096) ? 1 : segs);
  launch_qknorm_rope(x, ld, M, D, w, cs, sn, rpr, eps, c->stream, w_second, blocked);
}

void build_rope(ltx_ctx* c, int F, int H, int W) {
  if (c->rope_f == F && c->rope_h == H && c->rope_w == W && c->rope_cos.ptr) return;
  const ltx_config& g = c->cfg;
  const int D = g.num_heads * g.head_dim;
  const int half = D / 2;
  const int n_idx = std::max(1, D / 6);
  const int pad = std::max(0, half - n_idx * 3);
  const int64_t N = static_cast<int64_t>(F) * H * W;
  std::vector<float> cs(static_cast<size_t>(N) * half), sn(static_cast<size_t>(N) * half);
  std::vector<double> idx(n_idx);
  for (int i = 0; i < n_idx; ++i) {
    const double t = n_idx > 1 ? static_cast<double>(i) / (n_idx - 1) : 0.0;
    idx[i] = std::pow(static_cast<double>(g.rope_theta), t) * (M_PI / 2.0);
  }
  for (int f = 0; f < F; ++f) {
    const float ts = 8.0f, fi = static_cast<float>(f);
    const float st = std::max(fi * ts + (1.0f - ts), 0.0f), en = std::max((fi + 1.0f) * ts + (1.0f - ts), 0.0f);
    const float pt = ((st + en) / 2.0f) / 24.0f;
    for (int y = 0; y < H; ++y) {
      const float phh = static_cast<float>(y) * 32.0f + 16.0f;
      for (int x = 0; x < W; ++x) {
        const float pw = static_cast<float>(x) * 32.0f + 16.0f;
        const int64_t n = (static_cast<int64_t>(f) * H + y) * W + x;
        const double sc[3] = {static_cast<double>(pt) / g.max_pos[0] * 2.0 - 1.0,
                              static_cast<double>(phh) / g.max_pos[1] * 2.0 - 1.0,
                              static_cast<double>(pw) / g.max_pos[2] * 2.0 - 1.0};
        float* cr = &cs[static_cast<size_t>(n) * half];
        float* sr = &sn[static_cast<size_t>(n) * half];
        for (int p = 0; p < pad; ++p) { cr[p] = 1.0f; sr[p] = 0.0f; }
        for (int k = 0; k < n_idx; ++k)
          for (int d = 0; d < 3; ++d) {
            const int o = pad + k * 3 + d;
            if (o >= half) continue;
            const double a = idx[k] * sc[d];
            cr[o] = static_cast<float>(std::cos(a));
            sr[o] = static_cast<float>(std::sin(a));
          }
      }
    }
  }
  const size_t bytes = cs.size() * sizeof(float);
  c->rope_cos.reserve(bytes);
  c->rope_sin.reserve(bytes);
  LTX_CUDA(cudaMemcpyAsync(c->rope_cos.ptr, cs.data(), bytes, cudaMemcpyHostToDevice, c->stream));
  LTX_CUDA(cudaMemcpyAsync(c->rope_sin.ptr, sn.data(), bytes, cudaMemcpyHostToDevice, c->stream));
  LTX_CUDA(cudaStreamSynchronize(c->stream));
  c->rope_f = F; c->rope_h = H; c->rope_w = W;
}

int64_t round_up(int64_t v, int64_t m) { return (v + m - 1) / m * m; }

bool in_list(int v, const int32_t* lst, int n) {
  for (int i = 0; i < n; ++i)
    if (lst[i] == v) return true;
  return false;
}

}

TextCache& dit_prepare_text(ltx_ctx* c, TextCache* slots, int* rr, const TextProjW& src, const void* context, int context_dtype,
                            const int32_t* mask_dev, int B, int S, uint64_t key) {
  const ltx_config& g = c->cfg;
  const int D = src.D, L = g.num_layers, Cc = g.caption_channels;
  if (key != 0)
    for (int i = 0; i < 2; ++i)
      if (slots[i].key == key && slots[i].B == B && slots[i].S == S) return slots[i];
  int slot = -1;
  for (int i = 0; i < 2; ++i)
    if (slots[i].key == 0) { slot = i; break; }
  if (slot < 0) slot = ((*rr)++) & 1;
  TextCache& tc = slots[slot];
  const int64_t R = static_cast<int64_t>(B) * S;
  tc.key = key; tc.fingerprint = 0; tc.B = B; tc.S = S;
  tc.ldv = round_up(S, 8);
  tc.k.reserve(static_cast<size_t>(L) * R * D * 2);
  tc.vt.reserve(static_cast<size_t>(L) * D * B * tc.ldv * 2);
  cudaStream_t st = c->stream;
  const bf16* ctx_bf;
  if (context_dtype == LTX_BF16) {
    ctx_bf = reinterpret_cast<const bf16*>(context);
  } else {
    LTX_CHECK(context_dtype == LTX_F32, LTX_ERR_UNSUPPORTED, "context dtype must be bf16 or f32");
    LTX_CHECK((R * Cc) % 4 == 0, LTX_ERR_INVALID_ARGUMENT, "context size");
    c->ctx_in.reserve(static_cast<size_t>(R) * Cc * 2);
    {
      ProfScope ps(c, PROF_OTHER, 0.0, 6.0 * R * Cc);
      launch_cast_f32_bf16(reinterpret_cast<const float*>(context), c->ctx_in.as<bf16>(), R * Cc, st);
    }
    ctx_bf = c->ctx_in.as<bf16>();
  }
  c->c1.reserve(static_cast<size_t>(R) * D * 2);
  c->c2.reserve(static_cast<size_t>(R) * D * 2);
  LinearOpts o;
  o.split_k = true;
  GemmEpi e;
  e.mode = EPI_GELU_BF16; e.out = c->c1.ptr; e.ldo = D; e.bias = src.b_c1;
  linear(c, ctx_bf, Cc, src.w_c1, static_cast<int>(R), D, Cc, e, o);
  e.mode = EPI_BF16; e.out = c->c2.ptr; e.bias = src.b_c2;
  linear(c, c->c1.as<bf16>(), D, src.w_c2, static_cast<int>(R), D, D, e, o);
  for (int i = 0; i < L; ++i) {
    const AttnWeights& a = src.layer(src.user, i);
    bf16* kd = tc.k.as<bf16>() + static_cast<int64_t>(i) * R * D;
    bf16* vd = tc.vt.as<bf16>() + static_cast<int64_t>(i) * D * B * tc.ldv;
    GemmEpi ek;
    ek.mode = EPI_BF16; ek.out = kd; ek.ldo = D; ek.bias = a.bk;
    linear(c, c->c2.as<bf16>(), D, a.wk, static_cast<int>(R), D, D, ek, o);
    qknorm(c, kd, D, static_cast<int>(R), D, a.k_norm, nullptr, nullptr, 1, g.norm_eps);
    for (int b = 0; b < B; ++b)
      linear_vt(c, c->c2.as<bf16>() + static_cast<int64_t>(b) * S * D, S, 1, a.wv, a.bv, vd + b * tc.ldv, B * tc.ldv, tc.ldv,
                c->c1.as<bf16>(), o);
  }
  bool any_masked = false;
  if (mask_dev) {
    std::vector<int32_t> hm(static_cast<size_t>(R));
    LTX_CUDA(cudaMemcpyAsync(hm.data(), mask_dev, static_cast<size_t>(R) * 4, cudaMemcpyDeviceToHost, st));
    LTX_CUDA(cudaStreamSynchronize(st));
    for (int32_t v : hm) any_masked |= (v == 0);
  }
  tc.has_bias = any_masked;
  if (any_masked) {
    tc.bias.reserve(static_cast<size_t>(R) * 4);
    ProfScope ps(c, PROF_OTHER, 0.0, 8.0 * R);
    launch_mask_to_bias(mask_dev, tc.bias.as<float>(), static_cast<int>(R), st);
  }
  return tc;
}

namespace {
const AttnWeights& video_text_layer(const void* user, int i) { return static_cast<const ltx_ctx*>(user)->blocks[i].a2; }
TextCache& prepare_text(ltx_ctx* c, const void* context, int context_dtype, const int32_t* mask_dev, int B, int S,
                        uint64_t key) {
  TextProjW src;
  src.w_c1 = c->w_c1; src.w_c2 = c->w_c2; src.b_c1 = c->b_c1; src.b_c2 = c->b_c2;
  src.D = c->cfg.num_heads * c->cfg.head_dim; src.user = c; src.layer = video_text_layer;
  return dit_prepare_text(c, c->text, &c->text_rr, src, context, context_dtype, mask_dev, B, S, key);
}
}

void dit_build_rope(ltx_ctx* c, int F, int H, int W) { build_rope(c, F, H, W); }

void gemm_attach_workspace(ltx_ctx* c, GemmEpi& e) {
  constexpr size_t kCounters = 16384, kPartials = static_cast<size_t>(40) << 20;
  if (!c->gemm_ws.ptr) {
    c->gemm_ws.reserve(kCounters * 4 + kPartials);
    LTX_CUDA(cudaMemsetAsync(c->gemm_ws.ptr, 0, kCounters * 4, c->stream));
  }
  e.ws_counters = c->gemm_ws.as<unsigned int>();
  e.ws_counter_count = kCounters;
  e.ws = reinterpret_cast<float*>(c->gemm_ws.as<uint8_t>() + kCounters * 4);
  e.ws_bytes = kPartials;
}

void dit_clear_caches(ltx_ctx* c) {
  c->rope_f = c->rope_h = c->rope_w = 0;
  for (auto& t : c->text) { t.key = 0; t.fingerprint = 0; t.B = t.S = 0; }
  for (auto& t : c->av.text) { t.key = 0; t.fingerprint = 0; t.B = t.S = 0; }
  c->av.rope_ta = c->av.rope_f = c->av.rope_hw = 0;
}

void dit_finalize(ltx_ctx* c) {
  const ltx_config& g = c->cfg;
  LTX_CHECK(g.head_dim == 128, LTX_ERR_INVALID_CONFIGURATION, "head_dim must be 128");
  const int64_t D = static_cast<int64_t>(g.num_heads) * g.head_dim, FF = g.ffn_mult * D;
  LTX_CHECK(g.in_channels % 8 == 0 && g.caption_channels % 8 == 0 && g.out_channels % 8 == 0, LTX_ERR_INVALID_CONFIGURATION,
            "channel counts must be multiples of 8");
  c->w_patch = wlin(c, "patchify_proj.weight", D, g.in_channels);
  c->b_patch = wf(c, "patchify_proj.bias", D);
  c->adaln = adaln_w(c, "adaln_single", D, 6);
  c->w_c1 = wlin(c, "caption_projection.linear_1.weight", D, g.caption_channels);
  c->b_c1 = wf(c, "caption_projection.linear_1.bias", D);
  c->w_c2 = wlin(c, "caption_projection.linear_2.weight", D, D);
  c->b_c2 = wf(c, "caption_projection.linear_2.bias", D);
  c->sst_out = wf(c, "scale_shift_table", 2 * D);
  c->w_out = wlin(c, "proj_out.weight", g.out_channels, D);
  c->b_out = wf(c, "proj_out.bias", g.out_channels);
  c->blocks.assign(g.num_layers, BlockWeights());
  for (int i = 0; i < g.num_layers; ++i) {
    const std::string p = "transformer_blocks." + std::to_string(i) + ".";
    BlockWeights& b = c->blocks[i];
    b.sst = wf(c, p + "scale_shift_table", 6 * D);
    {
      const bf16* wq = wbf(c, p + "attn1.to_q.weight", D, D);
      const bf16* wk = wbf(c, p + "attn1.to_k.weight", D, D);
      const bf16* wv = wbf(c, p + "attn1.to_v.weight", D, D);
      const float* bq = wf(c, p + "attn1.to_q.bias", D);
      const float* bk = wf(c, p + "attn1.to_k.bias", D);
      const float* bvv = wf(c, p + "attn1.to_v.bias", D);
      bf16* wqkv = nullptr;
      float* bqkv = nullptr;
      LTX_CUDA(cudaMalloc(&wqkv, static_cast<size_t>(3) * D * D * 2));
      c->owned.push_back(wqkv);
      LTX_CUDA(cudaMalloc(&bqkv, static_cast<size_t>(3) * D * 4));
      c->owned.push_back(bqkv);
      const bf16* ws[3] = {wq, wk, wv};
      const float* bs[3] = {bq, bk, bvv};
      for (int t = 0; t < 3; ++t) {
        LTX_CUDA(cudaMemcpyAsync(wqkv + static_cast<size_t>(t) * D * D, ws[t], static_cast<size_t>(D) * D * 2, cudaMemcpyDeviceToDevice, c->stream));
        LTX_CUDA(cudaMemcpyAsync(bqkv + static_cast<size_t>(t) * D, bs[t], static_cast<size_t>(D) * 4, cudaMemcpyDeviceToDevice, c->stream));
      }
      LTX_CUDA(cudaStreamSynchronize(c->stream));
      for (const char* k : {"attn1.to_q.weight", "attn1.to_k.weight", "attn1.to_v.weight"}) {
        auto it = c->tensors.find(p + k);
        cudaFree(it->second.ptr);
        c->tensors.erase(it);
      }
      b.a1.wq.n = 3 * D; b.a1.wq.k = D; b.a1.wq.w = wqkv;
      b.a1.wv.n = D; b.a1.wv.k = D; b.a1.wv.w = wqkv + 2 * D * D;
      b.a1.bq = bqkv; b.a1.bk = bqkv + D; b.a1.bv = bqkv + 2 * D;
    }
    b.a1.wo = wlin(c, p + "attn1.to_out.weight", D, D);
    b.a1.bo = wf(c, p + "attn1.to_out.bias", D);
    b.a1.q_norm = wf(c, p + "attn1.q_norm.weight", D);
    b.a1.k_norm = wf(c, p + "attn1.k_norm.weight", D);
    b.a2.wq = wlin(c, p + "attn2.to_q.weight", D, D);
    b.a2.bq = wf(c, p + "attn2.to_q.bias", D);
    b.a2.wk = wlin(c, p + "attn2.to_k.weight", D, D);
    b.a2.bk = wf(c, p + "attn2.to_k.bias", D);
    b.a2.wv = wlin(c, p + "attn2.to_v.weight", D, D);
    b.a2.bv = wf(c, p + "attn2.to_v.bias", D);
    b.a2.wo = wlin(c, p + "attn2.to_out.weight", D, D);
    b.a2.bo = wf(c, p + "attn2.to_out.bias", D);
    b.a2.q_norm = wf(c, p + "attn2.q_norm.weight", D);
    b.a2.k_norm = wf(c, p + "attn2.k_norm.weight", D);
    b.w_in = wlin(c, p + "ff.project_in.proj.weight", FF, D);
    b.b_in = wf(c, p + "ff.project_in.proj.bias", FF);
    b.w_out = wlin(c, p + "ff.project_out.weight", D, FF);
    b.b_out = wf(c, p + "ff.project_out.bias", D);
  }
  c->scratch.reserve(64 * sizeof(double));
  c->dit_ready = true;
}

namespace {
void release_weight(ltx_ctx* c, const void* p) {
  for (auto it = c->tensors.begin(); it != c->tensors.end(); ++it)
    if (it->second.ptr == p) { cudaFree(it->second.ptr); c->tensors.erase(it); return; }
  for (auto it = c->owned.begin(); it != c->owned.end(); ++it)
    if (*it == p) { cudaFree(*it); c->owned.erase(it); return; }
}
}

void dit_quantize(ltx_ctx* c, int bits) {
  LTX_CHECK(c->dit_ready, LTX_ERR_WEIGHTS, "DiT weights not finalized");
  LTX_CHECK(bits == 8 || bits == 4, LTX_ERR_UNSUPPORTED, "quant_bits must be 16, 8 or 4");
  const ltx_config& g = c->cfg;
  const int D = g.num_heads * g.head_dim;
  std::vector<const void*> to_free;
  std::vector<LinearW*> coded;
  auto qf = [&](LinearW& w, int rows = 0) {
    const int N = rows ? rows : w.n, K = w.k;
    LTX_CHECK(w.fmt == LW_BF16, LTX_ERR_WEIGHTS, "quantisation needs bf16 weights");
    LTX_CHECK(K % 64 == 0, LTX_ERR_INVALID_CONFIGURATION, "quantisation needs every Linear input width to be a multiple of 64");
    uint8_t* q = nullptr;
    float *s = nullptr, *b = nullptr;
    const size_t qbytes = static_cast<size_t>(N) * K * bits / 8, sbytes = static_cast<size_t>(K / 64) * N * 4;
    LTX_CUDA(cudaMalloc(&q, qbytes));
    LTX_CUDA(cudaMalloc(&s, sbytes));
    LTX_CUDA(cudaMalloc(&b, sbytes));
    c->owned.push_back(q); c->owned.push_back(s); c->owned.push_back(b);
    launch_quantize(w.w, N, K, bits, q, s, b, c->stream);
    QuantW r;
    r.q = q; r.scales = s; r.biases = b; r.bits = bits; r.n = N; r.k = K;
    if (c->quant_materialise) {
      launch_dequantize_panel(r, const_cast<bf16*>(w.w), c->stream);
      LTX_CUDA(cudaStreamSynchronize(c->stream));
      for (void* ptr : {static_cast<void*>(q), static_cast<void*>(s), static_cast<void*>(b)}) {
        cudaFree(ptr);
        c->owned.erase(std::find(c->owned.begin(), c->owned.end(), ptr));
      }
      return;
    }
    LTX_CUDA(cudaStreamSynchronize(c->stream));
    to_free.push_back(w.w);
    w.fmt = LW_AFFINE; w.n = N; w.w = nullptr; w.q = r;
    coded.push_back(&w);
  };
  qf(c->w_patch); qf(c->w_c1); qf(c->w_c2); qf(c->w_out);
  for (auto& b : c->blocks) {
    qf(b.a1.wq, 2 * D);
    qf(b.a1.wv); qf(b.a1.wo);
    qf(b.a2.wq); qf(b.a2.wk); qf(b.a2.wv); qf(b.a2.wo);
    qf(b.w_in); qf(b.w_out);
  }
  if (c->av.ready) {
    AvWeights& a = c->av;
    qf(a.w_patch); qf(a.w_c1); qf(a.w_c2); qf(a.w_out);
    for (auto& b : a.blocks) {
      for (AttnWeights* w : {&b.aa1, &b.aa2, &b.a2v, &b.v2a}) { qf(w->wq); qf(w->wk); qf(w->wv); qf(w->wo); }
      qf(b.w_in); qf(b.w_out);
    }
  }
  c->quant_bits = bits;
  if (c->quant_materialise) return;
  for (const void* p : to_free) release_weight(c, p);
  size_t max_elems = 0;
  for (const LinearW* w : coded) max_elems = std::max(max_elems, static_cast<size_t>(w->n) * w->k);
  c->q_panel.reserve(max_elems * 2);
  for (LinearW* w : coded) w->q.scratch = c->q_panel.as<bf16>();
}

void dit_convert_fp8(ltx_ctx* c) {
  LTX_CHECK(c->dit_ready, LTX_ERR_WEIGHTS, "DiT weights not finalized");
  const ltx_config& g = c->cfg;
  const int D = g.num_heads * g.head_dim, FF = g.ffn_mult * D;
  LTX_CHECK(D % 16 == 0 && FF % 16 == 0, LTX_ERR_INVALID_CONFIGURATION, "FP8 mode needs Linear widths that are multiples of 16");
  std::vector<const void*> to_free;
  auto conv = [&](LinearW& w) {
    LTX_CHECK(w.fmt == LW_BF16, LTX_ERR_WEIGHTS, "FP8 conversion needs unquantised DiT weights");
    const int N = w.n, K = w.k;
    uint8_t* q = nullptr;
    float* s = nullptr;
    LTX_CUDA(cudaMalloc(&q, static_cast<size_t>(N) * K));
    LTX_CUDA(cudaMalloc(&s, static_cast<size_t>(N) * 4));
    c->owned.push_back(q); c->owned.push_back(s);
    launch_quantize_rows_fp8(w.w, K, N, K, q, s, c->stream);
    to_free.push_back(w.w);
    w.fmt = LW_E4M3; w.w = nullptr;
    w.q.q = q; w.q.scales = s; w.q.bits = 8; w.q.n = N; w.q.k = K;
  };
  for (auto& b : c->blocks) {
    conv(b.a1.wq);
    b.a1.wv = b.a1.wq;
    b.a1.wv.n = b.a1.wv.q.n = D;
    b.a1.wv.q.q += static_cast<size_t>(2) * D * D; b.a1.wv.q.scales += 2 * D;
    conv(b.a1.wo);
    conv(b.a2.wq); conv(b.a2.wk); conv(b.a2.wv); conv(b.a2.wo);
    conv(b.w_in); conv(b.w_out);
  }
  LTX_CUDA(cudaStreamSynchronize(c->stream));
  for (const void* p : to_free) release_weight(c, p);
}

void dit_forward_dev(ltx_ctx* c, const void* latent, int latent_dtype, const void* context, int context_dtype,
                     const float* timesteps_dev, int ts_per_token, const int32_t* mask_dev, int B, int N, int S, int F,
                     int H, int W, const ltx_dit_flags* flags, float* out_velocity_dev, int snapshot_block, int resume_block) {
  LTX_CHECK(c->dit_ready, LTX_ERR_WEIGHTS, "DiT weights not finalized");
  LTX_CHECK(B >= 1 && B <= 4 && N >= 1 && S >= 1, LTX_ERR_INVALID_ARGUMENT, "bad B/N/S");
  LTX_CHECK(static_cast<int64_t>(F) * H * W == N, LTX_ERR_INVALID_ARGUMENT, "N must equal F*H*W");
  LTX_CHECK(latent && context && timesteps_dev && out_velocity_dev, LTX_ERR_INVALID_ARGUMENT, "null tensor");
  if (c->precision == 32) {
    dit_forward_f32(c, latent, latent_dtype, context, context_dtype, timesteps_dev, ts_per_token, mask_dev, B, N, S, F, H, W, flags,
                    out_velocity_dev);
    return;
  }
  const ltx_config& g = c->cfg;
  const int D = g.num_heads * g.head_dim, FFD = g.ffn_mult * D, Hh = g.num_heads, L = g.num_layers;
  const int Cin = g.in_channels, Cout = g.out_channels;
  const int P = (c->dist.comm_world && c->dist.sp > 1) ? c->dist.sp : 1;
  LTX_CHECK(P == 1 || c->precision != 8, LTX_ERR_UNSUPPORTED, "FP8 mode has no sequence-parallel forward");
  LTX_CHECK(P == 1 || (B == 1 && N % P == 0 && Hh % P == 0), LTX_ERR_INVALID_ARGUMENT,
            "sequence parallelism needs B == 1 and N, num_heads divisible by sp_size");
  const int Nl = N / P, tok0 = (P > 1 ? c->dist.sp_rank : 0) * Nl;
  const int R = (P > 1) ? Nl : B * N;
  const int Nq = (P > 1) ? Nl : N;
  const int Csp = D / P, Hl = Hh / P;
  const float eps = g.norm_eps;
  cudaStream_t st = c->stream;
  LinearOpts o;
  o.split_k = true;
  ltx_dit_flags noflags = {};
  noflags.cross_attn_scale = 1.0f;
  if (!flags) flags = &noflags;
  LTX_CHECK(flags->n_stg_blocks >= 0 && flags->n_stg_blocks <= LTX_MAX_FLAG_BLOCKS && flags->n_cas_blocks >= 0 &&
                flags->n_cas_blocks <= LTX_MAX_FLAG_BLOCKS,
            LTX_ERR_INVALID_ARGUMENT, "bad flag block counts");

  const int64_t ldv = round_up(N, 8);
  c->x.reserve(static_cast<size_t>(R) * D * 4);
  c->xb.reserve(static_cast<size_t>(R) * D * 2);
  c->h.reserve(static_cast<size_t>(R) * D * 2);
  c->qk.reserve(static_cast<size_t>(R) * 2 * D * 2);
  c->vt.reserve(static_cast<size_t>(D) * B * ldv * 2);
  c->att.reserve(static_cast<size_t>(R) * D * 2);
  c->q2.reserve(static_cast<size_t>(R) * D * 2);
  c->ffh.reserve(static_cast<size_t>(R) * FFD * 2);
  const int TR = ts_per_token ? R : B;
  c->se.reserve(static_cast<size_t>(TR) * 256 * 4);
  c->t1.reserve(static_cast<size_t>(TR) * D * 4);
  c->emb.reserve(static_cast<size_t>(TR) * D * 4);
  c->ada.reserve(static_cast<size_t>(TR) * 6 * D * 4);
  float* x = c->x.as<float>();
  bf16* xb = c->xb.as<bf16>();
  bf16* h = c->h.as<bf16>();
  bf16* qk = c->qk.as<bf16>();
  bf16* vt = c->vt.as<bf16>();
  bf16* att = c->att.as<bf16>();
  bf16* q2 = c->q2.as<bf16>();
  bf16* ffh = c->ffh.as<bf16>();
  float* ada = c->ada.as<float>();
  float* emb = c->emb.as<float>();
  const int64_t blk = static_cast<int64_t>(Nl) * Csp;
  bf16 *qsend = nullptr, *ksend = nullptr, *vsend = nullptr, *qrecv = nullptr, *krecv = nullptr, *vrecv = nullptr,
       *osend = nullptr, *orecv = nullptr, *vt_sp = nullptr;
  bool p2p = false;
  bf16* peer_base[LTX_MAX_PEERS] = {};
  const int me = c->dist.sp_rank;
  if (P > 1) {
    p2p = dist_p2p_ensure(c, static_cast<size_t>(4) * P * blk * 2);
    c->sp_vt.reserve(static_cast<size_t>(Csp) * ldv * 2);
    c->sp_vel.reserve(static_cast<size_t>(Nl) * Cout * 4);
    vt_sp = c->sp_vt.as<bf16>();
    if (p2p) {
      for (int r = 0; r < P; ++r) peer_base[r] = reinterpret_cast<bf16*>(c->dist.p2p_peer[r]);
      qrecv = peer_base[me]; krecv = qrecv + P * blk; vrecv = krecv + P * blk; orecv = vrecv + P * blk;
      osend = orecv;
    } else {
      c->sp_send.reserve(static_cast<size_t>(3) * P * blk * 2);
      c->sp_recv.reserve(static_cast<size_t>(3) * P * blk * 2);
      qsend = c->sp_send.as<bf16>(); ksend = qsend + P * blk; vsend = ksend + P * blk;
      qrecv = c->sp_recv.as<bf16>(); krecv = qrecv + P * blk; vrecv = krecv + P * blk;
      osend = qsend;
      orecv = qrecv;
    }
  }

  build_rope(c, F, H, W);
  TextCache& tc = prepare_text(c, context, context_dtype, mask_dev, B, S, flags->context_key);
  const float* key_bias = tc.has_bias ? tc.bias.as<float>() : nullptr;
  const float* cos_l = c->rope_cos.as<float>() + static_cast<int64_t>(tok0) * (D / 2);
  const float* sin_l = c->rope_sin.as<float>() + static_cast<int64_t>(tok0) * (D / 2);
  const int rope_period = (P > 1) ? Nl : N;
  const int rows_per_b = ts_per_token ? 1 : rope_period;

  const bf16* lat_bf;
  if (latent_dtype == LTX_BF16) {
    lat_bf = reinterpret_cast<const bf16*>(latent);
  } else {
    LTX_CHECK(latent_dtype == LTX_F32, LTX_ERR_UNSUPPORTED, "latent dtype must be bf16 or f32");
    c->lat_in.reserve(static_cast<size_t>(B) * N * Cin * 2);
    {
      ProfScope ps(c, PROF_OTHER, 0.0, 6.0 * B * N * Cin);
      launch_cast_f32_bf16(reinterpret_cast<const float*>(latent), c->lat_in.as<bf16>(), static_cast<int64_t>(B) * N * Cin, st);
    }
    lat_bf = c->lat_in.as<bf16>();
  }
  lat_bf += static_cast<int64_t>(tok0) * Cin;
  if (resume_block < 0) {
    GemmEpi e;
    e.mode = EPI_BF16; e.out = xb; e.ldo = D; e.bias = c->b_patch;
    linear(c, lat_bf, Cin, c->w_patch, R, D, Cin, e, o);
    ProfScope ps(c, PROF_OTHER, 0.0, 6.0 * R * D);
    launch_cast_bf16_f32(xb, x, static_cast<int64_t>(R) * D, st);
  } else {
    LTX_CHECK(resume_block < L && c->snap_x.ptr && c->snap_rows >= R, LTX_ERR_INVALID_ARGUMENT, "no matching snapshot to resume from");
    ProfScope ps(c, PROF_OTHER, 0.0, 14.0 * R * D, 2);
    LTX_CUDA(cudaMemcpyAsync(x, c->snap_x.ptr, static_cast<size_t>(R) * D * 4, cudaMemcpyDeviceToDevice, st));
    launch_cast_f32_bf16(x, xb, static_cast<int64_t>(R) * D, st);
  }
  if (!ts_per_token) {
    adaln_single(c, c->adaln, c->se.as<float>(), c->t1.as<float>(), emb, ada, B, timesteps_dev, g.timestep_scale_multiplier);
  } else {
    bf16* se_bf = reinterpret_cast<bf16*>(c->se.ptr);
    {
      ProfScope ps(c, PROF_OTHER, 0.0, 4.0 * R + 512.0 * R);
      launch_sincos_embed(timesteps_dev + tok0, g.timestep_scale_multiplier, nullptr, R, 256, st, se_bf);
    }
    adaln_single_rows(c, c->adaln, se_bf, R, reinterpret_cast<bf16*>(c->t1.ptr), emb, ada, 6 * D, o);
  }

  const int64_t ada_ld = 6 * static_cast<int64_t>(D);
  for (int i = (resume_block > 0 ? resume_block : 0); i < L; ++i) {
    const BlockWeights& bw = c->blocks[i];
    if (i == snapshot_block) {
      c->snap_x.reserve(static_cast<size_t>(R) * D * 4);
      c->snap_rows = R;
      ProfScope ps(c, PROF_OTHER, 0.0, 8.0 * R * D);
      LTX_CUDA(cudaMemcpyAsync(c->snap_x.ptr, x, static_cast<size_t>(R) * D * 4, cudaMemcpyDeviceToDevice, st));
    }
    const bool flagged = in_list(i, flags->stg_blocks, flags->n_stg_blocks);
    const bool skip_sa = flagged && flags->skip_self_attn;
    const bool skip_ff = flagged && flags->skip_ff;
    const float cas = in_list(i, flags->cas_blocks, flags->n_cas_blocks) ? flags->cross_attn_scale : 1.0f;
    if (!skip_sa) {
      norm_mod(c, x, h, R, D, bw.sst, bw.sst + D, ada, ada + D, ada_ld, rows_per_b, eps, 0);
      const bool packed_qkv = bw.a1.wq.fmt != LW_AFFINE;
      const bool fused_qkv = P == 1 && (B == 1 || ldv == N) && packed_qkv && D % 32 == 0;
      GemmEpi e;
      e.mode = EPI_BF16; e.out = qk; e.ldo = 2 * D; e.bias = bw.a1.bq;
      if (fused_qkv) {
        e.tsplit_col = 2 * D; e.out_t = vt; e.ldt = B * ldv;
        LinearOpts ow;
        ow.tile_n = 256;
        linear(c, h, D, bw.a1.wq, R, 3 * D, D, e, ow);
      } else if (P == 1) {
        linear(c, h, D, bw.a1.wq, R, 2 * D, D, e, o);
      }
      if (P == 1) {
        for (int b = 0; b < B && !fused_qkv; ++b)
          linear_vt(c, h + static_cast<int64_t>(b) * N * D, N, 1, bw.a1.wv, bw.a1.bv, vt + b * ldv, B * ldv, ldv, q2, o);
        qknorm(c, qk, 2 * D, R, D, bw.a1.q_norm, cos_l, sin_l, rope_period, eps, bw.a1.k_norm);
        attention(c, qk, 2 * D, qk + D, 2 * D, vt, ldv, nullptr, att, D, B, Hh, N, N, D);
      } else {
        GemmEpi ev;
        ev.mode = EPI_BF16; ev.out = p2p ? vrecv : vsend; ev.ldo = Csp; ev.bias = bw.a1.bv; ev.col_block = Csp; ev.col_block_stride = blk;
        QkOut qo;
        qo.out[0] = qsend; qo.out[1] = ksend; qo.heads_per_block = Hl; qo.block_stride = blk; qo.ld = Csp;
        PeerTable ot = {};
        if (p2p) {
          ev.use_col_ptrs = 1;
          qo.use_peer = 1;
          for (int d = 0; d < P; ++d) {
            qo.peer[0].p[d] = peer_base[d] + static_cast<int64_t>(0 * P + me) * blk;
            qo.peer[1].p[d] = peer_base[d] + static_cast<int64_t>(1 * P + me) * blk;
            ev.col_ptrs.p[d] = peer_base[d] + static_cast<int64_t>(2 * P + me) * blk;
            ot.p[d] = peer_base[d] + static_cast<int64_t>(3 * P + me) * blk;
          }
        }
        if (packed_qkv) {
          GemmEpi eqkv = ev;
          eqkv.out = qk; eqkv.ldo = 2 * D; eqkv.bias = bw.a1.bq;
          eqkv.col_block_from = 2 * D; eqkv.blocked_out = ev.out; eqkv.blocked_ld = Csp;
          linear(c, h, D, bw.a1.wq, R, 3 * D, D, eqkv, o);
        } else {
          linear(c, h, D, bw.a1.wq, R, 2 * D, D, e, o);
          linear(c, h, D, bw.a1.wv, R, D, D, ev, o);
        }
        qknorm(c, qk, 2 * D, R, D, bw.a1.q_norm, cos_l, sin_l, rope_period, eps, bw.a1.k_norm, &qo);
        if (p2p) {
          ProfScope ps(c, PROF_COMM, 0.0, 3.0 * 2.0 * P * blk * 2.0);
          dist_p2p_barrier(c, 0);
        } else {
          ProfScope ps(c, PROF_COMM, 0.0, 3.0 * 2.0 * P * blk * 2.0);
          const void* sb[3] = {qsend, ksend, vsend};
          void* rb[3] = {qrecv, krecv, vrecv};
          dist_all_to_all_sp(c, sb, rb, 3, static_cast<size_t>(blk) * 2);
        }
        {
          ProfScope ps(c, PROF_OTHER, 0.0, 4.0 * N * Csp);
          launch_transpose_bf16(vrecv, Csp, N, Csp, vt_sp, ldv, st);
        }
        if (p2p) {
          attention(c, qrecv, Csp, krecv, Csp, vt_sp, ldv, nullptr, osend, Csp, 1, Hl, N, N, Csp, &ot, Nl);
          ProfScope ps(c, PROF_COMM, 0.0, 2.0 * P * blk * 2.0);
          dist_p2p_barrier(c, 1);
        } else {
          attention(c, qrecv, Csp, krecv, Csp, vt_sp, ldv, nullptr, osend, Csp, 1, Hl, N, N, Csp);
          ProfScope ps(c, PROF_COMM, 0.0, 2.0 * P * blk * 2.0);
          const void* sb[1] = {osend};
          void* rb[1] = {orecv};
          dist_all_to_all_sp(c, sb, rb, 1, static_cast<size_t>(blk) * 2);
        }
      }
      GemmEpi eo;
      eo.mode = EPI_GATE_RESID; eo.resid = x; eo.ldr = D; eo.bias = bw.a1.bo;
      eo.gate_a = ada + 2 * D; eo.gate_b = bw.sst + 2 * D; eo.gate_ld = ada_ld; eo.rows_per_gate = rows_per_b;
      eo.shadow = xb; eo.lds = D;
      if (P == 1) {
        linear(c, att, D, bw.a1.wo, R, D, D, eo, o);
      } else {
        LinearOpts ok = o;
        ok.a_kblock = Csp; ok.a_kblock_stride = blk;
        linear(c, orecv, Csp, bw.a1.wo, R, D, D, eo, ok);
      }
    }
    {
      GemmEpi e;
      e.mode = EPI_BF16; e.out = q2; e.ldo = D; e.bias = bw.a2.bq;
      linear(c, xb, D, bw.a2.wq, R, D, D, e, o);
      qknorm(c, q2, D, R, D, bw.a2.q_norm, nullptr, nullptr, 1, eps);
      const bf16* k2 = tc.k.as<bf16>() + static_cast<int64_t>(i) * B * S * D;
      const bf16* v2 = tc.vt.as<bf16>() + static_cast<int64_t>(i) * D * B * tc.ldv;
      attention(c, q2, D, k2, D, v2, tc.ldv, key_bias, att, D, B, Hh, Nq, S, D);
      GemmEpi eo;
      eo.mode = EPI_GATE_RESID; eo.resid = x; eo.ldr = D; eo.bias = bw.a2.bo; eo.scale = cas;
      const bool next_needs_shadow = skip_ff && (i + 1 < L) &&
                                     in_list(i + 1, flags->stg_blocks, flags->n_stg_blocks) && flags->skip_self_attn;
      if (next_needs_shadow) { eo.shadow = xb; eo.lds = D; }
      linear(c, att, D, bw.a2.wo, R, D, D, eo, o);
    }
    if (!skip_ff) {
      norm_mod(c, x, h, R, D, bw.sst + 3 * D, bw.sst + 4 * D, ada + 3 * D, ada + 4 * D, ada_ld, rows_per_b, eps, 0);
      GemmEpi e;
      e.mode = EPI_GELU_BF16; e.out = ffh; e.ldo = FFD; e.bias = bw.b_in;
      linear(c, h, D, bw.w_in, R, FFD, D, e, o);
      GemmEpi eo;
      eo.mode = EPI_GATE_RESID; eo.resid = x; eo.ldr = D; eo.bias = bw.b_out;
      eo.gate_a = ada + 5 * D; eo.gate_b = bw.sst + 5 * D; eo.gate_ld = ada_ld; eo.rows_per_gate = rows_per_b;
      const bool next_needs_shadow =
          (i + 1 < L) && in_list(i + 1, flags->stg_blocks, flags->n_stg_blocks) && flags->skip_self_attn;
      if (next_needs_shadow) { eo.shadow = xb; eo.lds = D; }
      linear(c, ffh, FFD, bw.w_out, R, D, FFD, eo, o);
    }
  }
  norm_mod(c, x, h, R, D, c->sst_out, c->sst_out + D, emb, emb, D, rows_per_b, eps, 1);
  GemmEpi e;
  e.mode = EPI_F32; e.out = (P > 1) ? c->sp_vel.ptr : out_velocity_dev; e.ldo = Cout; e.bias = c->b_out;
  linear(c, h, D, c->w_out, R, Cout, D, e, o);
  if (P > 1) {
    ProfScope ps(c, PROF_COMM, 0.0, 4.0 * N * Cout);
    dist_allgather_sp(c, c->sp_vel.ptr, out_velocity_dev, static_cast<size_t>(Nl) * Cout * 4);
  }
}

}
```

ltx-video-swift-mlx_b200/csrc/gemm2.cu:

```cuda
#include "gemm_epilogue.cuh"
#include "ltx_internal.h"
#include "ptx.cuh"

namespace ltx {

namespace {

constexpr int BM2 = 128;
constexpr int BK2 = 64;
constexpr int G2_THREADS = 192;
constexpr int G2_BN_MAX = 256;
constexpr uint32_t G2_A_BYTES = BM2 * BK2 * 2;
constexpr uint32_t G2_B_STRIDE = (G2_BN_MAX / 2) * BK2 * 2;
constexpr int G2_KSUB = 2;
constexpr int G2_STAGES = 3;
constexpr uint32_t G2_A_STAGE = G2_KSUB * G2_A_BYTES, G2_B_STAGE = G2_KSUB * G2_B_STRIDE;
constexpr size_t G2_SMEM = 1024 + G2_STAGES * (G2_A_STAGE + G2_B_STAGE) + (2 * G2_STAGES + 4) * 8 + 16 + 128 + 4 * EPI_STAGE_BYTES;

template <int MODE, bool FP8>
__global__ void __cluster_dims__(2, 1, 1) __launch_bounds__(G2_THREADS, 1)
gemm_bf16_2cta(const __grid_constant__ CUtensorMap tmA, const __grid_constant__ CUtensorMap tmB, int M, int N, int K, int BN,
               int a_kblock, const GemmEpi ep, const float* sa, const float* sb) {
  constexpr int AK = FP8 ? 2 * BK2 : BK2;
  extern __shared__ uint8_t smem_raw[];
  uint8_t* smem = reinterpret_cast<uint8_t*>((reinterpret_cast<uintptr_t>(smem_raw) + 1023) & ~static_cast<uintptr_t>(1023));
  uint8_t* sA = smem;
  uint8_t* sB = smem + G2_STAGES * G2_A_STAGE;
  uint64_t* full = reinterpret_cast<uint64_t*>(sB + G2_STAGES * G2_B_STAGE);
  uint64_t* empty = full + G2_STAGES;
  uint64_t* tfull = empty + G2_STAGES;
  uint64_t* tempty = tfull + 2;
  uint32_t* tmem_slot = reinterpret_cast<uint32_t*>(tempty + 2);
  float* epi_stage = reinterpret_cast<float*>((reinterpret_cast<uintptr_t>(tmem_slot + 4) + 127) & ~static_cast<uintptr_t>(127));

  const int warp = threadIdx.x >> 5, lane = threadIdx.x & 31;
  const uint32_t rank = cluster_ctarank();
  const bool leader = rank == 0;
  const int cluster_id = blockIdx.x >> 1, num_clusters = gridDim.x >> 1;
  const int num_mp = (M + 2 * BM2 - 1) / (2 * BM2);
  const int num_n = (N + BN - 1) / BN;
  const int num_tiles = num_mp * num_n;
  const int num_k = (K + G2_KSUB * AK - 1) / (G2_KSUB * AK);
  const int half_bn = BN >> 1;
  const uint32_t b_bytes = static_cast<uint32_t>(half_bn) * BK2 * 2;

  if (warp == 0 && lane == 0) {
    tma_prefetch_desc(&tmA);
    tma_prefetch_desc(&tmB);
    for (int i = 0; i < G2_STAGES; ++i) {
      mbar_init(&full[i], 2);
      mbar_init(&empty[i], 1);
    }
    for (int i = 0; i < 2; ++i) {
      mbar_init(&tfull[i], 1);
      mbar_init(&tempty[i], 8);
    }
    fence_mbar_init();
  }
  if (warp == 1) tmem_alloc_2cta<512>(tmem_slot);
  tc_fence_before();
  cluster_sync_all();
  tc_fence_after();
  const uint32_t tmem_base = *tmem_slot;
  griddep_launch();
  griddep_wait();

  if (warp == 0) {
    if (lane == 0) {
      int stage = 0;
      uint32_t phase = 0;
      for (int tile = cluster_id; tile < num_tiles; tile += num_clusters) {
        const int mp = tile % num_mp, n_blk = tile / num_mp;
        const int m0 = (mp * 2 + static_cast<int>(rank)) * BM2;
        const int n0 = n_blk * BN + static_cast<int>(rank) * half_bn;
        for (int kb = 0; kb < num_k; ++kb) {
          mbar_wait(&empty[stage], phase ^ 1);
          if (leader) mbar_arrive_expect_tx(&full[stage], 2 * G2_KSUB * (G2_A_BYTES + b_bytes));
          else mbar_arrive_remote(&full[stage], 0);
#pragma unroll
          for (int ks = 0; ks < G2_KSUB; ++ks) {
            const int k0 = (kb * G2_KSUB + ks) * AK;
            if (a_kblock > 0)
              tma_load_3d_2sm(sA + stage * G2_A_STAGE + ks * G2_A_BYTES, &tmA, &full[stage], k0 % a_kblock, m0, k0 / a_kblock);
            else
              tma_load_2d_2sm(sA + stage * G2_A_STAGE + ks * G2_A_BYTES, &tmA, &full[stage], k0, m0);
            tma_load_2d_2sm(sB + stage * G2_B_STAGE + ks * G2_B_STRIDE, &tmB, &full[stage], k0, n0);
          }
          if (++stage == G2_STAGES) { stage = 0; phase ^= 1; }
        }
      }
    }
  } else if (warp == 1) {
    if (leader && lane == 0) {
      const uint32_t idesc = FP8 ? umma_idesc_e4m3(2 * BM2, BN) : umma_idesc_bf16(2 * BM2, BN);
      const uint64_t a_desc0 = umma_desc_sw128(smem_u32(sA)), b_desc0 = umma_desc_sw128(smem_u32(sB));
      int stage = 0;
      uint32_t phase = 0;
      int t = 0;
      for (int tile = cluster_id; tile < num_tiles; tile += num_clusters, ++t) {
        const int as = t & 1;
        const uint32_t aphase = (t >> 1) & 1;
        mbar_wait(&tempty[as], aphase ^ 1);
        tc_fence_after();
        const uint32_t d_tmem = tmem_base + as * G2_BN_MAX;
        for (int kb = 0; kb < num_k; ++kb) {
          mbar_wait(&full[stage], phase);
          tc_fence_after();
          const uint64_t a_desc = a_desc0 + static_cast<uint64_t>(stage) * (G2_A_STAGE >> 4);
          const uint64_t b_desc = b_desc0 + static_cast<uint64_t>(stage) * (G2_B_STAGE >> 4);
#pragma unroll
          for (int ks = 0; ks < G2_KSUB; ++ks)
#pragma unroll
            for (int k = 0; k < BK2 / 16; ++k) {
              const uint64_t ad = a_desc + ((ks * G2_A_BYTES + k * 32) >> 4), bd = b_desc + ((ks * G2_B_STRIDE + k * 32) >> 4);
              if (FP8) umma_f8_2cta(d_tmem, ad, bd, idesc, (kb | ks | k) != 0 ? 1u : 0u);
              else umma_bf16_2cta(d_tmem, ad, bd, idesc, (kb | ks | k) != 0 ? 1u : 0u);
            }
          umma_commit_2cta(&empty[stage]);
          if (++stage == G2_STAGES) { stage = 0; phase ^= 1; }
        }
        umma_commit_2cta(&tfull[as]);
      }
    }
  } else {
    const int q = warp & 3;
    int t = 0;
    for (int tile = cluster_id; tile < num_tiles; tile += num_clusters, ++t) {
      const int mp = tile % num_mp, n_blk = tile / num_mp;
      const int as = t & 1;
      const uint32_t aphase = (t >> 1) & 1;
      mbar_wait(&tfull[as], aphase);
      tc_fence_after();
      const uint32_t taddr = tmem_base + (static_cast<uint32_t>(q * 32) << 16) + as * G2_BN_MAX;
      epilogue_tile<MODE, FP8>(taddr, BN, epi_stage + (warp - 2) * (EPI_STAGE_BYTES / 4), lane,
                               (mp * 2 + static_cast<int>(rank)) * BM2 + q * 32, n_blk * BN, M, N, ep, sa, sb);
      tc_fence_before();
      __syncwarp();
      if (lane == 0) mbar_arrive_remote(&tempty[as], 0);
    }
  }
  tc_fence_before();
  cluster_sync_all();
  if (warp == 1) {
    tc_fence_after();
    tmem_dealloc_2cta<512>(tmem_base);
  }
}

template <int MODE, bool FP8 = false>
void launch2(const CUtensorMap& tmA, const CUtensorMap& tmB, int M, int N, int K, int BN, int a_kblock, const GemmEpi& epi,
             cudaStream_t stream, const float* sa = nullptr, const float* sb = nullptr) {
  auto kern = gemm_bf16_2cta<MODE, FP8>;
  ensure_dyn_smem(kern, G2_SMEM);
  const int tiles = ((M + 2 * BM2 - 1) / (2 * BM2)) * ((N + BN - 1) / BN);
  const int clusters = device_sm_count() / 2;
  const int grid = 2 * (tiles < clusters ? tiles : clusters);
  launch_pdl(PDL_GEMM, kern, dim3(grid), dim3(G2_THREADS), G2_SMEM, stream, tmA, tmB, M, N, K, BN, a_kblock, epi, sa, sb);
}

template <bool FP8>
void launch2_mode(const CUtensorMap& tmA, const CUtensorMap& tmB, int M, int N, int K, int bn, int a_kblock, const GemmEpi& epi,
                  cudaStream_t stream, const float* sa, const float* sb) {
  switch (epi.mode) {
    case EPI_BF16: launch2<EPI_BF16, FP8>(tmA, tmB, M, N, K, bn, a_kblock, epi, stream, sa, sb); break;
    case EPI_GELU_BF16: launch2<EPI_GELU_BF16, FP8>(tmA, tmB, M, N, K, bn, a_kblock, epi, stream, sa, sb); break;
    case EPI_GATE_RESID: launch2<EPI_GATE_RESID, FP8>(tmA, tmB, M, N, K, bn, a_kblock, epi, stream, sa, sb); break;
    case EPI_F32: launch2<EPI_F32, FP8>(tmA, tmB, M, N, K, bn, a_kblock, epi, stream, sa, sb); break;
    case EPI_SILU_BF16: launch2<EPI_SILU_BF16, FP8>(tmA, tmB, M, N, K, bn, a_kblock, epi, stream, sa, sb); break;
    default: LTX_CHECK(false, 2, "bad GEMM epilogue mode");
  }
}

void check_tsplit(const GemmEpi& epi, int bn) {
  LTX_CHECK(epi.tsplit_col == 0 || (epi.mode == EPI_BF16 && bn % 32 == 0 && epi.tsplit_col % 32 == 0 && epi.out_t != nullptr &&
                                    epi.ldt % 8 == 0 && epi.col_block == 0),
            2, "GEMM: transposed-column output needs the bf16 epilogue, a tile width and split column that are multiples of 32");
}

}

int gemm2_fit_tile_width(int M, int N) {
  const int clusters = device_sm_count() / 2;
  const int num_mp = (M + 255) / 256;
  int best = 256;
  double best_cost = 1e30;
  for (int bn = 256; bn >= 64; bn -= 16) {
    const long long tiles = static_cast<long long>(num_mp) * ((N + bn - 1) / bn);
    const long long waves = (tiles + clusters - 1) / clusters;
    const double cost = static_cast<double>(waves) * (bn + 100.0);
    if (cost < best_cost - 1e-9) { best_cost = cost; best = bn; }
  }
  return best;
}

void launch_gemm_2cta(const bf16* A, int64_t lda, const bf16* B, int64_t ldb, int M, int N, int K, const GemmEpi& epi,
                      cudaStream_t stream, int force_bn, int a_kblock, int64_t a_kblock_stride) {
  int bn = force_bn ? force_bn : gemm2_fit_tile_width(M, N);
  LTX_CHECK(bn >= 64 && bn <= 256 && bn % 16 == 0, 2, "2-CTA GEMM: tile width must be a multiple of 16 in [64, 256]");
  check_tsplit(epi, bn);
  CUtensorMap tmA;
  if (a_kblock > 0) {
    LTX_CHECK(a_kblock % BK2 == 0 && K % a_kblock == 0 && lda == a_kblock, 2, "GEMM: bad K-blocked A layout");
    tmA = make_tmap_3d(A, a_kblock, M, K / a_kblock, lda, a_kblock_stride, 64, BM2);
  } else {
    tmA = make_tmap_2d(A, M, K, lda, BM2);
  }
  CUtensorMap tmB = make_tmap_2d(B, N, K, ldb, bn / 2);
  launch2_mode<false>(tmA, tmB, M, N, K, bn, a_kblock, epi, stream, nullptr, nullptr);
}

void launch_gemm_fp8(const uint8_t* A, int64_t lda, const float* sa, const uint8_t* B, int64_t ldb, const float* sb, int M, int N,
                     int K, const GemmEpi& epi, cudaStream_t stream, int force_bn) {
  LTX_CHECK(M > 0 && N > 0 && K > 0, 2, "GEMM: empty problem");
  LTX_CHECK(K % 16 == 0 && lda % 16 == 0 && ldb % 16 == 0 && lda >= K && ldb >= K, 2,
            "FP8 GEMM: K and the row pitches must be multiples of 16 bytes");
  LTX_CHECK(sa != nullptr && sb != nullptr && (reinterpret_cast<uintptr_t>(sb) & 15) == 0, 2,
            "FP8 GEMM: row scales of both operands needed (sb 16-byte aligned)");
  LTX_CHECK(epi.col_block == 0 && epi.transpose_out == 0, 2, "FP8 GEMM: no column-blocked or transposed-row output");
  if (epi.mode == EPI_GATE_RESID) {
    LTX_CHECK(epi.resid != nullptr && epi.ldr % 4 == 0, 2, "GEMM: residual epilogue needs fp32 resid with ld % 4 == 0");
    LTX_CHECK(epi.shadow == nullptr || epi.lds % 4 == 0, 2, "GEMM: shadow ld must be a multiple of 4");
  } else {
    LTX_CHECK(epi.out != nullptr, 2, "GEMM: missing output");
    LTX_CHECK(epi.ldo % (epi.mode == EPI_F32 ? 4 : 8) == 0, 2, "GEMM: output ld alignment");
  }
  const int bn = force_bn ? force_bn : gemm2_fit_tile_width(M, N);
  LTX_CHECK(bn >= 64 && bn <= 256 && bn % 16 == 0, 2, "2-CTA GEMM: tile width must be a multiple of 16 in [64, 256]");
  check_tsplit(epi, bn);
  const CUtensorMap tmA = make_tmap_u8_sw128(A, M, K, lda, BM2);
  const CUtensorMap tmB = make_tmap_u8_sw128(B, N, K, ldb, bn / 2);
  launch2_mode<true>(tmA, tmB, M, N, K, bn, 0, epi, stream, sa, sb);
}

}
```

ltx-video-swift-mlx_b200/csrc/ltx_internal.h:

```cpp
#pragma once
#include <cuda.h>
#include <cuda_bf16.h>
#include <cuda_runtime.h>
#include <stdint.h>

#include <stdexcept>
#include <string>

namespace ltx {

typedef __nv_bfloat16 bf16;

struct LtxError : public std::runtime_error {
  int code;
  LtxError(int c, const std::string& m) : std::runtime_error(m), code(c) {}
};

#define LTX_CHECK(cond, code, msg)                                                                  \
  do {                                                                                              \
    if (!(cond)) throw ::ltx::LtxError((code), std::string(msg) + " [" #cond "] at " __FILE__ ":" + \
                                                   std::to_string(__LINE__));                       \
  } while (0)
#define LTX_CUDA(expr)                                                                                       \
  do {                                                                                                       \
    cudaError_t _e = (expr);                                                                                 \
    if (_e != cudaSuccess)                                                                                   \
      throw ::ltx::LtxError(3, std::string("CUDA error: ") + cudaGetErrorString(_e) + " in " #expr " at " + \
                                   __FILE__ ":" + std::to_string(__LINE__));                                 \
  } while (0)

bool pdl_enabled(int cls = 0);
enum { PDL_GEMM = 0, PDL_ROWS = 1, PDL_ATTN = 2, PDL_VAE = 3 };
template <typename... KArgs, typename... Args>
inline void launch_pdl(int cls, void (*kern)(KArgs...), dim3 grid, dim3 block, size_t smem, cudaStream_t stream, Args&&... args) {
  cudaLaunchConfig_t cfg = {};
  cfg.gridDim = grid;
  cfg.blockDim = block;
  cfg.dynamicSmemBytes = smem;
  cfg.stream = stream;
  cudaLaunchAttribute at[1];
  at[0].id = cudaLaunchAttributeProgrammaticStreamSerialization;
  at[0].val.programmaticStreamSerializationAllowed = 1;
  cfg.attrs = at;
  cfg.numAttrs = pdl_enabled(cls) ? 1 : 0;
  LTX_CUDA(cudaLaunchKernelEx(&cfg, kern, static_cast<KArgs>(args)...));
}

CUtensorMap make_tmap_2d(const void* base, uint64_t rows, uint64_t cols, uint64_t ld, uint32_t box_rows,
                         uint32_t box_cols = 64);
CUtensorMap make_tmap_thwc(const void* base, uint64_t T, uint64_t H, uint64_t W, uint64_t C, uint32_t bt, uint32_t bh,
                           uint32_t bw);
CUtensorMap make_tmap_3d(const void* base, uint64_t d0, uint64_t d1, uint64_t d2, uint64_t stride1, uint64_t stride2,
                         uint32_t box0, uint32_t box1);
int device_sm_count();
void ensure_dyn_smem(const void* kernel, size_t bytes);
template <typename K>
inline void ensure_dyn_smem(K* kernel, size_t bytes) { ensure_dyn_smem(reinterpret_cast<const void*>(kernel), bytes); }

enum EpiMode : int {
  EPI_BF16 = 0,
  EPI_GELU_BF16 = 1,
  EPI_GATE_RESID = 2,
  EPI_F32 = 3,
  EPI_SILU_BF16 = 4,
};

constexpr int LTX_MAX_PEERS = 8;
struct PeerTable {
  void* p[LTX_MAX_PEERS];
};

struct GemmEpi {
  int mode = EPI_BF16;
  void* out = nullptr;
  int64_t ldo = 0;
  const float* bias = nullptr;
  int bias_per_row = 0;
  float* resid = nullptr;
  int64_t ldr = 0;
  const float* gate_a = nullptr;
  const float* gate_b = nullptr;
  int64_t gate_ld = 0;
  int rows_per_gate = 1;
  bf16* shadow = nullptr;
  int64_t lds = 0;
  float scale = 1.0f;
  int col_block = 0;
  int64_t col_block_stride = 0;
  int use_col_ptrs = 0;
  PeerTable col_ptrs = {};
  int col_block_from = 0;
  void* blocked_out = nullptr;
  int64_t blocked_ld = 0;
  int tsplit_col = 0;
  bf16* out_t = nullptr;
  int64_t ldt = 0;
  int transpose_out = 0;
  int t_item_rows = 0;
  int64_t t_item_ld = 0;
  float* ws = nullptr;
  size_t ws_bytes = 0;
  unsigned int* ws_counters = nullptr;
  size_t ws_counter_count = 0;
};

void launch_gemm(const bf16* A, int64_t lda, const bf16* B, int64_t ldb, int M, int N, int K, const GemmEpi& epi,
                 cudaStream_t stream, int force_bn = 0, int a_kblock = 0, int64_t a_kblock_stride = 0, int allow_skinny = 0);
bool gemm_skinny_eligible(int64_t lda, int64_t ldb, int M, int N, int K, const GemmEpi& epi, int a_kblock, int max_rows = 32);
void launch_gemm_skinny(const bf16* A, int64_t lda, const bf16* W, int64_t ldb, int M, int N, int K, const GemmEpi& epi,
                        cudaStream_t stream);
int gemm_fit_tile_width(int M, int N);
bool gemm_swapab_eligible(int64_t lda, int64_t ldb, int M, int N, int K, const GemmEpi& epi);
void launch_gemm_swapab(const bf16* A, int64_t lda, const bf16* W, int64_t ldb, int M, int N, int K, const GemmEpi& epi,
                        cudaStream_t stream, int a_kblock = 0, int64_t a_kblock_stride = 0);
void launch_gemm_2cta(const bf16* A, int64_t lda, const bf16* B, int64_t ldb, int M, int N, int K, const GemmEpi& epi,
                      cudaStream_t stream, int force_bn, int a_kblock, int64_t a_kblock_stride);
int gemm2_fit_tile_width(int M, int N);
void launch_gemm_fp8(const uint8_t* A, int64_t lda, const float* sa, const uint8_t* B, int64_t ldb, const float* sb, int M, int N,
                     int K, const GemmEpi& epi, cudaStream_t stream, int force_bn = 0);
void launch_quantize_rows_fp8(const bf16* x, int64_t ld, int M, int K, uint8_t* q, float* s, cudaStream_t stream);
struct QuantW {
  const uint8_t* q = nullptr;
  const float* scales = nullptr;
  const float* biases = nullptr;
  int bits = 0, n = 0, k = 0;
  bf16* scratch = nullptr;
};
void launch_gemm_q(const bf16* A, int64_t lda, const QuantW& W, int M, int N, int K, const GemmEpi& epi, cudaStream_t stream,
                   int force_bn = 0, int a_kblock = 0, int64_t a_kblock_stride = 0);
bool gemm_q_uses_panel(const QuantW& W, int M);
void launch_quantize(const bf16* w, int N, int K, int bits, uint8_t* q, float* scales, float* biases, cudaStream_t s);
void launch_dequantize(const QuantW& W, bf16* w, cudaStream_t s);
void launch_dequantize_panel(const QuantW& W, bf16* w, cudaStream_t s);
CUtensorMap make_tmap_u8(const void* base, uint64_t rows, uint64_t row_bytes, uint32_t box_rows, uint32_t box_bytes);
CUtensorMap make_tmap_u8_sw128(const void* base, uint64_t rows, uint64_t cols, uint64_t row_bytes, uint32_t box_rows);
void launch_transpose_bf16(const bf16* in, int64_t ld_in, int R, int C, bf16* out, int64_t ld_out, cudaStream_t s);

void launch_attention(const bf16* Q, int64_t ldq, const bf16* K, int64_t ldk, const bf16* Vt, int64_t ldvb,
                      const float* key_bias, bf16* O, int64_t ldo, int B, int H, int Nq, int Nk, int D, float scale,
                      cudaStream_t stream, const PeerTable* o_blocks = nullptr, int rows_per_block = 0);

void launch_rmsnorm_mod(const float* x, bf16* out, int M, int D, const float* tbl_shift, const float* tbl_scale,
                        const float* ada_shift, const float* ada_scale, int64_t ada_ld, int rows_per_mod, float eps,
                        int layernorm, cudaStream_t s);
struct QkOut {
  bf16* out[2] = {nullptr, nullptr};
  int heads_per_block = 0;
  int64_t block_stride = 0, ld = 0;
  int use_peer = 0;
  PeerTable peer[2] = {};
};
void launch_qknorm_rope(bf16* x, int64_t ld, int M, int D, const float* w, const float* cosb, const float* sinb,
                        int rows_per_rope, float eps, cudaStream_t s, const float* w_second = nullptr,
                        const QkOut* blocked = nullptr);
void launch_cast_f32_bf16(const float* in, bf16* out, int64_t n, cudaStream_t s);
void launch_cast_bf16_f32(const bf16* in, float* out, int64_t n, cudaStream_t s);
void launch_gemv(const bf16* W, const float* bias, const float* x, float* y, int M, int O, int I, int silu_in,
                 cudaStream_t s);
void launch_mask_to_bias(const int32_t* mask, float* bias, int n, cudaStream_t s);
void launch_scale_f32(float* x, float a, int64_t n, cudaStream_t s);
void launch_audio_cfg_euler(float* lat, const float* v_cond, const float* v_uncond, float cfg_scale, float dt, int64_t n,
                            cudaStream_t s);
void launch_sincos_embed(const float* sigma, float mult, float* out, int M, int dim, cudaStream_t s, bf16* out_bf16 = nullptr);
void launch_silu_cast(const float* in, bf16* out, int64_t n, cudaStream_t s);
void launch_fill_token_timesteps(float* ts, int n, int period, int frozen, const float* sigma_dev, cudaStream_t s);
void launch_patchify(const float* latent, bf16* tok_bf16, float* tok_f32, int C, int T, cudaStream_t s);
void launch_unpatchify(const float* tok, float* latent, int C, int T, cudaStream_t s);
void launch_transpose_slice(const float* in, int64_t ld_in, int rows, int cols, float* out, cudaStream_t s);
struct GuidedEulerArgs {
  float* latent;
  const float* v_cond;
  const float* v_uncond;
  const float* v_stg;
  float* v_prev;
  int use_prev;
  float* v_out;
  size_t n;
  float cfg, phi, stg, ge_gamma, sigma, sigma_next;
  double* scratch;
  size_t period = 0, frozen = 0;
};
void launch_guided_euler(const GuidedEulerArgs& a, cudaStream_t s);
void launch_fill_normal_bf16(bf16* p, int64_t n, float std, float mean, uint64_t seed, cudaStream_t s);
void launch_fill_normal_f32(float* p, int64_t n, float std, float mean, uint64_t seed, cudaStream_t s);

struct ConvEpi {
  int mode;
  float* out;
  const float* bias;
  const float* resid;
  int Cin;
  int t_shift = 0;
  bf16* next_pad = nullptr;
  const float* next_scale = nullptr;
  const float* next_shift = nullptr;
  int next_tshift = 1;
  int no_clip = 0;
};
bool conv3d_wants_tap_split(int H, int W, int Cin, int Cout);
struct ConvPlan {
  int bn;
  int pair;
  int slab;
  int bt, bh, bw;
  int ksplit;
};
ConvPlan conv3d_plan(int T, int H, int W, int Cin, int Cout, int mode, int ntaps, bool scratch_ok, int sm_count, bool pair_on,
                     bool slab_on);
bool conv3d_pair_default();
bool conv3d_slab_default();
void launch_conv3d(const bf16* x_pad, const bf16* w, int T, int H, int W, int Cin, int Cout, const ConvEpi& epi,
                   cudaStream_t s, int ntaps = 27, float* splitk_scratch = nullptr, size_t splitk_scratch_bytes = 0);
enum { VAE_PAD_CAUSAL = 1, VAE_PAD_ZERO_HW = 2, VAE_PAD_ZERO_T = 4 };
void launch_vae_halo_fill(bf16* pad_vol, int T, int H, int W, int C, int pad, cudaStream_t s);
void launch_vae_prep(const float* x, bf16* out, int T, int H, int W, int C, int mode, const float* a, const float* b,
                     int pad, cudaStream_t s);

}
```

Before: 25.99.

## Chain attention output projection and cross-attn Q projection in one persistent GEMM

Adds a two-phase persistent 2-CTA GEMM kernel. Its second phase (the cross-attention Q projection) starts loading A rows once per-row-tile readiness counters show the first phase (the self-attention output projection with gated residual, which writes the bf16 shadow) has finished those rows. The DiT block uses it when the weights are bf16 and there are more than 512 rows, removing a kernel boundary and the tail underutilisation between the two GEMMs. This adds spin-waits on global counters (deadlock risk if not all clusters are resident, handled by an occupancy query), a counter reset done by the last block, and a jointly chosen tile width.

```diff
diff --git a/include/ltxcuda.h b/include/ltxcuda.h
--- a/include/ltxcuda.h
+++ b/include/ltxcuda.h
@@ -195,6 +195,8 @@
                         int K, int col_from, int col_block, int64_t block_stride, int force_bn);
 int ltx_op_gemm_resid(ltx_ctx* ctx, const void* A, const void* B, const float* bias, float* x, const float* gate_a,
                       const float* gate_b, void* shadow, int M, int N, int K, float scale);
+int ltx_op_gemm_chain(ltx_ctx* ctx, const void* A0, const void* B0, const float* bias0, const void* B1, const float* bias1, float* x,
+                      const float* gate_a, const float* gate_b, void* shadow, void* out, int M, int N0, int K, int N1);
 int ltx_op_gemm_skinny(ltx_ctx* ctx, const void* A, const void* B, const float* bias, void* out, float* x, const float* gate_a,
                        const float* gate_b, int rows_per_gate, int M, int N, int K, int mode, int items, int64_t vt_item_ld);
 int ltx_op_quantize(ltx_ctx* ctx, const void* w_bf16, int N, int K, int bits, void* q_out, float* scales_out, float* biases_out);
diff --git a/ltx-video-swift-mlx_b200/_lib.py b/ltx-video-swift-mlx_b200/_lib.py
--- a/ltx-video-swift-mlx_b200/_lib.py
+++ b/ltx-video-swift-mlx_b200/_lib.py
@@ -104,6 +104,7 @@
     "ltx_op_gemm": (_I, [_P, _P, _P, _P, _P, _I, _I, _I, _I, _I]),
     "ltx_op_gemm_blocked": (_I, [_P, _P, _P, _P, _P, _P, _I, _I, _I, _I, _I, C.c_int64, _I]),
     "ltx_op_gemm_resid": (_I, [_P, _P, _P, _P, _P, _P, _P, _P, _I, _I, _I, _F]),
+    "ltx_op_gemm_chain": (_I, [_P, _P, _P, _P, _P, _P, _P, _P, _P, _P, _P, _I, _I, _I, _I]),
     "ltx_op_gemm_skinny": (_I, [_P, _P, _P, _P, _P, _P, _P, _P, _I, _I, _I, _I, _I, _I, C.c_int64]),
     "ltx_op_quantize": (_I, [_P, _P, _I, _I, _I, _P, _P, _P]),
     "ltx_op_dequantize": (_I, [_P, _P, _P, _P, _I, _I, _I, _P]),
diff --git a/ltx-video-swift-mlx_b200/csrc/api.cu b/ltx-video-swift-mlx_b200/csrc/api.cu
--- a/ltx-video-swift-mlx_b200/csrc/api.cu
+++ b/ltx-video-swift-mlx_b200/csrc/api.cu
@@ -1241,6 +1241,24 @@
   });
 }
 
+int ltx_op_gemm_chain(ltx_ctx* c, const void* A0, const void* B0, const float* bias0, const void* B1, const float* bias1, float* x,
+                      const float* gate_a, const float* gate_b, void* shadow, void* out, int M, int N0, int K, int N1) {
+  return guarded(c, [&] {
+    LTX_CHECK(A0 && B0 && B1 && x && shadow && out, LTX_ERR_INVALID_ARGUMENT, "bad chained GEMM arguments");
+    GemmCall g0, g1;
+    g0.A = reinterpret_cast<const bf16*>(A0); g0.lda = K; g0.B = reinterpret_cast<const bf16*>(B0); g0.ldb = K; g0.N = N0; g0.K = K;
+    g0.epi.mode = EPI_GATE_RESID; g0.epi.bias = bias0; g0.epi.resid = x; g0.epi.ldr = N0; g0.epi.gate_a = gate_a;
+    g0.epi.gate_b = gate_b; g0.epi.gate_ld = 0; g0.epi.rows_per_gate = M > 0 ? M : 1;
+    g0.epi.shadow = reinterpret_cast<bf16*>(shadow); g0.epi.lds = N0;
+    g1.A = reinterpret_cast<const bf16*>(shadow); g1.lda = N0; g1.B = reinterpret_cast<const bf16*>(B1); g1.ldb = N0; g1.N = N1;
+    g1.K = N0;
+    g1.epi.mode = EPI_BF16; g1.epi.bias = bias1; g1.epi.out = out; g1.epi.ldo = N1;
+    LTX_CHECK(K == N0, LTX_ERR_INVALID_ARGUMENT, "chained GEMM: both products run over the same K (K == N0)");
+    launch_gemm_2cta_chain(g0, g1, M, gemm_chain_counters(c), c->stream);
+    c->launches++;
+  });
+}
+
 int ltx_op_gemm_skinny(ltx_ctx* c, const void* A, const void* B, const float* bias, void* out, float* x, const float* gate_a,
                        const float* gate_b, int rows_per_gate, int M, int N, int K, int mode, int items, int64_t vt_item_ld) {
   return guarded(c, [&] {
diff --git a/ltx-video-swift-mlx_b200/csrc/ctx.h b/ltx-video-swift-mlx_b200/csrc/ctx.h
--- a/ltx-video-swift-mlx_b200/csrc/ctx.h
+++ b/ltx-video-swift-mlx_b200/csrc/ctx.h
@@ -221,6 +221,7 @@
   int quant_materialise = 0;
   ltx::DevBuf q_panel;
   ltx::DevBuf gemm_ws;
+  ltx::DevBuf gemm_chain;
   std::vector<void*> owned;
   bool dit_ready = false;
   std::vector<ltx::BlockWeights> blocks;
@@ -269,6 +270,7 @@
 
 namespace ltx {
 void gemm_attach_workspace(ltx_ctx* c, GemmEpi& e);
+unsigned int* gemm_chain_counters(ltx_ctx* c);
 struct ProfScope {
   ltx_ctx* c;
   ProfRec r;
@@ -300,6 +302,8 @@
   int64_t a_kblock_stride = 0;
 };
 void linear(ltx_ctx* c, const bf16* A, int64_t lda, const LinearW& W, int M, int N, int K, const GemmEpi& e, const LinearOpts& o);
+void linear_chain(ltx_ctx* c, const bf16* A0, int64_t lda0, const LinearW& W0, int N0, int K0, const GemmEpi& e0, const bf16* A1,
+                  int64_t lda1, const LinearW& W1, int N1, int K1, const GemmEpi& e1, int M, const LinearOpts& o);
 void linear_vt(ltx_ctx* c, const bf16* A, int rows, int items, const LinearW& W, const float* bias, bf16* out, int64_t ld_out,
                int64_t item_ld, bf16* tmp, const LinearOpts& o);
 void attention(ltx_ctx* c, const bf16* Q, int64_t ldq, const bf16* K, int64_t ldk, const bf16* Vt, int64_t ldv, const float* bias,
diff --git a/ltx-video-swift-mlx_b200/csrc/dit.cu b/ltx-video-swift-mlx_b200/csrc/dit.cu
--- a/ltx-video-swift-mlx_b200/csrc/dit.cu
+++ b/ltx-video-swift-mlx_b200/csrc/dit.cu
@@ -41,6 +41,23 @@
     ProfScope ps(c, PROF_GEMM, 2.0 * M * N * K, static_cast<double>(M) * K + static_cast<double>(N) * K + 2.0 * M * N);
     launch_gemm_fp8(q, K, s, W.q.q, W.q.k, W.q.scales, M, N, K, e, c->stream, o.tile_n);
   }
+}
+
+void linear_chain(ltx_ctx* c, const bf16* A0, int64_t lda0, const LinearW& W0, int N0, int K0, const GemmEpi& e0, const bf16* A1,
+                  int64_t lda1, const LinearW& W1, int N1, int K1, const GemmEpi& e1, int M, const LinearOpts& o) {
+  if (W0.fmt != LW_BF16 || W1.fmt != LW_BF16 || M <= 512 || o.tile_n != 0 || o.a_kblock != 0) {
+    linear(c, A0, lda0, W0, M, N0, K0, e0, o);
+    linear(c, A1, lda1, W1, M, N1, K1, e1, o);
+    return;
+  }
+  LTX_CHECK(W0.k == K0 && N0 >= 1 && N0 <= W0.n && W1.k == K1 && N1 >= 1 && N1 <= W1.n, LTX_ERR_INVALID_ARGUMENT,
+            "Linear: weight shape mismatch");
+  ProfScope ps(c, PROF_GEMM, 2.0 * M * (static_cast<double>(N0) * K0 + static_cast<double>(N1) * K1),
+               gemm_bytes(M, N0, K0) + gemm_bytes(M, N1, K1));
+  GemmCall g0, g1;
+  g0.A = A0; g0.lda = lda0; g0.B = W0.w; g0.ldb = K0; g0.N = N0; g0.K = K0; g0.epi = e0;
+  g1.A = A1; g1.lda = lda1; g1.B = W1.w; g1.ldb = K1; g1.N = N1; g1.K = K1; g1.epi = e1;
+  launch_gemm_2cta_chain(g0, g1, M, gemm_chain_counters(c), c->stream);
 }
 
 void linear_vt(ltx_ctx* c, const bf16* A, int rows, int items, const LinearW& W, const float* bias, bf16* out, int64_t ld_out,
@@ -298,6 +315,15 @@
   e.ws_counter_count = kCounters;
   e.ws = reinterpret_cast<float*>(c->gemm_ws.as<uint8_t>() + kCounters * 4);
   e.ws_bytes = kPartials;
+}
+
+unsigned int* gemm_chain_counters(ltx_ctx* c) {
+  if (!c->gemm_chain.ptr) {
+    const size_t bytes = (GEMM_CHAIN_ROW_TILES + 1) * sizeof(unsigned int);
+    c->gemm_chain.reserve(bytes);
+    LTX_CUDA(cudaMemsetAsync(c->gemm_chain.ptr, 0, bytes, c->stream));
+  }
+  return c->gemm_chain.as<unsigned int>();
 }
 
 void dit_clear_caches(ltx_ctx* c) {
@@ -620,6 +646,9 @@
     const bool skip_sa = flagged && flags->skip_self_attn;
     const bool skip_ff = flagged && flags->skip_ff;
     const float cas = in_list(i, flags->cas_blocks, flags->n_cas_blocks) ? flags->cross_attn_scale : 1.0f;
+    GemmEpi eq2;
+    eq2.mode = EPI_BF16; eq2.out = q2; eq2.ldo = D; eq2.bias = bw.a2.bq;
+    bool q2_done = false;
     if (!skip_sa) {
       norm_mod(c, x, h, R, D, bw.sst, bw.sst + D, ada, ada + D, ada_ld, rows_per_b, eps, 0);
       const bool packed_qkv = bw.a1.wq.fmt != LW_AFFINE;
@@ -695,7 +724,8 @@
       eo.gate_a = ada + 2 * D; eo.gate_b = bw.sst + 2 * D; eo.gate_ld = ada_ld; eo.rows_per_gate = rows_per_b;
       eo.shadow = xb; eo.lds = D;
       if (P == 1) {
-        linear(c, att, D, bw.a1.wo, R, D, D, eo, o);
+        linear_chain(c, att, D, bw.a1.wo, D, D, eo, xb, D, bw.a2.wq, D, D, eq2, R, o);
+        q2_done = true;
       } else {
         LinearOpts ok = o;
         ok.a_kblock = Csp; ok.a_kblock_stride = blk;
@@ -703,9 +733,7 @@
       }
     }
     {
-      GemmEpi e;
-      e.mode = EPI_BF16; e.out = q2; e.ldo = D; e.bias = bw.a2.bq;
-      linear(c, xb, D, bw.a2.wq, R, D, D, e, o);
+      if (!q2_done) linear(c, xb, D, bw.a2.wq, R, D, D, eq2, o);
       qknorm(c, q2, D, R, D, bw.a2.q_norm, nullptr, nullptr, 1, eps);
       const bf16* k2 = tc.k.as<bf16>() + static_cast<int64_t>(i) * B * S * D;
       const bf16* v2 = tc.vt.as<bf16>() + static_cast<int64_t>(i) * D * B * tc.ldv;
@@ -721,13 +749,13 @@
       norm_mod(c, x, h, R, D, bw.sst + 3 * D, bw.sst + 4 * D, ada + 3 * D, ada + 4 * D, ada_ld, rows_per_b, eps, 0);
       GemmEpi e;
       e.mode = EPI_GELU_BF16; e.out = ffh; e.ldo = FFD; e.bias = bw.b_in;
-      linear(c, h, D, bw.w_in, R, FFD, D, e, o);
       GemmEpi eo;
       eo.mode = EPI_GATE_RESID; eo.resid = x; eo.ldr = D; eo.bias = bw.b_out;
       eo.gate_a = ada + 5 * D; eo.gate_b = bw.sst + 5 * D; eo.gate_ld = ada_ld; eo.rows_per_gate = rows_per_b;
       const bool next_needs_shadow =
           (i + 1 < L) && in_list(i + 1, flags->stg_blocks, flags->n_stg_blocks) && flags->skip_self_attn;
       if (next_needs_shadow) { eo.shadow = xb; eo.lds = D; }
+      linear(c, h, D, bw.w_in, R, FFD, D, e, o);
       linear(c, ffh, FFD, bw.w_out, R, D, FFD, eo, o);
     }
   }
diff --git a/ltx-video-swift-mlx_b200/csrc/gemm2.cu b/ltx-video-swift-mlx_b200/csrc/gemm2.cu
--- a/ltx-video-swift-mlx_b200/csrc/gemm2.cu
+++ b/ltx-video-swift-mlx_b200/csrc/gemm2.cu
@@ -1,3 +1,5 @@
+#include <atomic>
+
 #include "gemm_epilogue.cuh"
 #include "ltx_internal.h"
 #include "ptx.cuh"
@@ -17,10 +19,45 @@
 constexpr uint32_t G2_A_STAGE = G2_KSUB * G2_A_BYTES, G2_B_STAGE = G2_KSUB * G2_B_STRIDE;
 constexpr size_t G2_SMEM = 1024 + G2_STAGES * (G2_A_STAGE + G2_B_STAGE) + (2 * G2_STAGES + 4) * 8 + 16 + 128 + 4 * EPI_STAGE_BYTES;
 
-template <int MODE, bool FP8>
+struct G2Phase {
+  int M, N, K, BN, a_kblock;
+  GemmEpi ep;
+};
+struct G2Params {
+  CUtensorMap tmA[2], tmB[2];
+  G2Phase ph[2];
+  const float* sa;
+  const float* sb;
+  unsigned int* ready;
+};
+
+__device__ __forceinline__ void rows_publish(unsigned int* ctr) {
+  asm volatile("red.release.gpu.global.add.u32 [%0], 1;" ::"l"(ctr) : "memory");
+}
+__device__ __forceinline__ void rows_wait(const unsigned int* ctr, unsigned int target) {
+  uint32_t spins = 0;
+  for (;;) {
+    unsigned int v;
+    asm volatile("ld.acquire.gpu.global.u32 %0, [%1];" : "=r"(v) : "l"(ctr) : "memory");
+    if (v >= target) break;
+    if (++spins > (1u << 26)) {
+      printf("ltxcuda: chained GEMM row-tile wait timeout block %d (seen %u of %u)\n", blockIdx.x, v, target);
+      __trap();
+    }
+  }
+  asm volatile("fence.proxy.async.global;" ::: "memory");
+}
+
+template <int NPH>
+__device__ __forceinline__ void tile_pos(int tile, int num_mp, int num_n, int& mp, int& n_blk) {
+  if (NPH == 1) { mp = tile % num_mp; n_blk = tile / num_mp; }
+  else { mp = tile / num_n; n_blk = tile % num_n; }
+}
+
+template <int MODE0, int MODE1, bool FP8>
 __global__ void __cluster_dims__(2, 1, 1) __launch_bounds__(G2_THREADS, 1)
-gemm_bf16_2cta(const __grid_constant__ CUtensorMap tmA, const __grid_constant__ CUtensorMap tmB, int M, int N, int K, int BN,
-               int a_kblock, const GemmEpi ep, const float* sa, const float* sb) {
+gemm_bf16_2cta(const __grid_constant__ G2Params p) {
+  constexpr int NPH = MODE1 < 0 ? 1 : 2;
   constexpr int AK = FP8 ? 2 * BK2 : BK2;
   extern __shared__ uint8_t smem_raw[];
   uint8_t* smem = reinterpret_cast<uint8_t*>((reinterpret_cast<uintptr_t>(smem_raw) + 1023) & ~static_cast<uintptr_t>(1023));
@@ -37,16 +74,14 @@
   const uint32_t rank = cluster_ctarank();
   const bool leader = rank == 0;
   const int cluster_id = blockIdx.x >> 1, num_clusters = gridDim.x >> 1;
-  const int num_mp = (M + 2 * BM2 - 1) / (2 * BM2);
-  const int num_n = (N + BN - 1) / BN;
-  const int num_tiles = num_mp * num_n;
-  const int num_k = (K + G2_KSUB * AK - 1) / (G2_KSUB * AK);
-  const int half_bn = BN >> 1;
-  const uint32_t b_bytes = static_cast<uint32_t>(half_bn) * BK2 * 2;
+  const unsigned int rows_target = 4u * static_cast<unsigned int>((p.ph[0].N + p.ph[0].BN - 1) / p.ph[0].BN);
 
   if (warp == 0 && lane == 0) {
-    tma_prefetch_desc(&tmA);
-    tma_prefetch_desc(&tmB);
+#pragma unroll
+    for (int ip = 0; ip < NPH; ++ip) {
+      tma_prefetch_desc(&p.tmA[ip]);
+      tma_prefetch_desc(&p.tmB[ip]);
+    }
     for (int i = 0; i < G2_STAGES; ++i) {
       mbar_init(&full[i], 2);
       mbar_init(&empty[i], 1);
@@ -69,74 +104,128 @@
     if (lane == 0) {
       int stage = 0;
       uint32_t phase = 0;
-      for (int tile = cluster_id; tile < num_tiles; tile += num_clusters) {
-        const int mp = tile % num_mp, n_blk = tile / num_mp;
-        const int m0 = (mp * 2 + static_cast<int>(rank)) * BM2;
-        const int n0 = n_blk * BN + static_cast<int>(rank) * half_bn;
-        for (int kb = 0; kb < num_k; ++kb) {
-          mbar_wait(&empty[stage], phase ^ 1);
-          if (leader) mbar_arrive_expect_tx(&full[stage], 2 * G2_KSUB * (G2_A_BYTES + b_bytes));
-          else mbar_arrive_remote(&full[stage], 0);
-#pragma unroll
-          for (int ks = 0; ks < G2_KSUB; ++ks) {
-            const int k0 = (kb * G2_KSUB + ks) * AK;
-            if (a_kblock > 0)
-              tma_load_3d_2sm(sA + stage * G2_A_STAGE + ks * G2_A_BYTES, &tmA, &full[stage], k0 % a_kblock, m0, k0 / a_kblock);
-            else
-              tma_load_2d_2sm(sA + stage * G2_A_STAGE + ks * G2_A_BYTES, &tmA, &full[stage], k0, m0);
-            tma_load_2d_2sm(sB + stage * G2_B_STAGE + ks * G2_B_STRIDE, &tmB, &full[stage], k0, n0);
+      int g = cluster_id, base = 0;
+#pragma unroll
+      for (int ip = 0; ip < NPH; ++ip) {
+        const G2Phase& ph = p.ph[ip];
+        const CUtensorMap* tmA = &p.tmA[ip];
+        const CUtensorMap* tmB = &p.tmB[ip];
+        const int num_mp = (ph.M + 2 * BM2 - 1) / (2 * BM2);
+        const int num_n = (ph.N + ph.BN - 1) / ph.BN;
+        const int num_tiles = num_mp * num_n;
+        const int num_k = (ph.K + G2_KSUB * AK - 1) / (G2_KSUB * AK);
+        const int half_bn = ph.BN >> 1;
+        const uint32_t b_bytes = static_cast<uint32_t>(half_bn) * BK2 * 2;
+        const int pre = ip == 1 ? (num_k < G2_STAGES ? num_k : G2_STAGES) : 0;
+        for (; g < base + num_tiles; g += num_clusters) {
+          const int tile = g - base;
+          int mp, n_blk;
+          tile_pos<NPH>(tile, num_mp, num_n, mp, n_blk);
+          const int m0 = (mp * 2 + static_cast<int>(rank)) * BM2;
+          const int n0 = n_blk * ph.BN + static_cast<int>(rank) * half_bn;
+          auto load_a = [&](int st, int kb) {
+#pragma unroll
+            for (int ks = 0; ks < G2_KSUB; ++ks) {
+              const int k0 = (kb * G2_KSUB + ks) * AK;
+              if (ph.a_kblock > 0)
+                tma_load_3d_2sm(sA + st * G2_A_STAGE + ks * G2_A_BYTES, tmA, &full[st], k0 % ph.a_kblock, m0, k0 / ph.a_kblock);
+              else
+                tma_load_2d_2sm(sA + st * G2_A_STAGE + ks * G2_A_BYTES, tmA, &full[st], k0, m0);
+            }
+          };
+          const int stage0 = stage;
+          for (int kb = 0; kb < num_k; ++kb) {
+            mbar_wait(&empty[stage], phase ^ 1);
+            if (leader) mbar_arrive_expect_tx(&full[stage], 2 * G2_KSUB * (G2_A_BYTES + b_bytes));
+            else mbar_arrive_remote(&full[stage], 0);
+            if (kb >= pre) load_a(stage, kb);
+#pragma unroll
+            for (int ks = 0; ks < G2_KSUB; ++ks)
+              tma_load_2d_2sm(sB + stage * G2_B_STAGE + ks * G2_B_STRIDE, tmB, &full[stage], (kb * G2_KSUB + ks) * AK, n0);
+            if (kb + 1 == pre) {
+              rows_wait(p.ready + mp * 2 + static_cast<int>(rank), rows_target);
+              for (int j = 0; j < pre; ++j) load_a((stage0 + j) % G2_STAGES, j);
+            }
+            if (++stage == G2_STAGES) { stage = 0; phase ^= 1; }
           }
-          if (++stage == G2_STAGES) { stage = 0; phase ^= 1; }
         }
+        base += num_tiles;
       }
     }
   } else if (warp == 1) {
     if (leader && lane == 0) {
-      const uint32_t idesc = FP8 ? umma_idesc_e4m3(2 * BM2, BN) : umma_idesc_bf16(2 * BM2, BN);
       const uint64_t a_desc0 = umma_desc_sw128(smem_u32(sA)), b_desc0 = umma_desc_sw128(smem_u32(sB));
       int stage = 0;
       uint32_t phase = 0;
       int t = 0;
-      for (int tile = cluster_id; tile < num_tiles; tile += num_clusters, ++t) {
-        const int as = t & 1;
-        const uint32_t aphase = (t >> 1) & 1;
-        mbar_wait(&tempty[as], aphase ^ 1);
-        tc_fence_after();
-        const uint32_t d_tmem = tmem_base + as * G2_BN_MAX;
-        for (int kb = 0; kb < num_k; ++kb) {
-          mbar_wait(&full[stage], phase);
+      int g = cluster_id, base = 0;
+#pragma unroll
+      for (int ip = 0; ip < NPH; ++ip) {
+        const G2Phase& ph = p.ph[ip];
+        const int num_tiles = ((ph.M + 2 * BM2 - 1) / (2 * BM2)) * ((ph.N + ph.BN - 1) / ph.BN);
+        const int num_k = (ph.K + G2_KSUB * AK - 1) / (G2_KSUB * AK);
+        const uint32_t idesc = FP8 ? umma_idesc_e4m3(2 * BM2, ph.BN) : umma_idesc_bf16(2 * BM2, ph.BN);
+        for (; g < base + num_tiles; g += num_clusters, ++t) {
+          const int as = t & 1;
+          const uint32_t aphase = (t >> 1) & 1;
+          mbar_wait(&tempty[as], aphase ^ 1);
           tc_fence_after();
-          const uint64_t a_desc = a_desc0 + static_cast<uint64_t>(stage) * (G2_A_STAGE >> 4);
-          const uint64_t b_desc = b_desc0 + static_cast<uint64_t>(stage) * (G2_B_STAGE >> 4);
-#pragma unroll
-          for (int ks = 0; ks < G2_KSUB; ++ks)
-#pragma unroll
-            for (int k = 0; k < BK2 / 16; ++k) {
-              const uint64_t ad = a_desc + ((ks * G2_A_BYTES + k * 32) >> 4), bd = b_desc + ((ks * G2_B_STRIDE + k * 32) >> 4);
-              if (FP8) umma_f8_2cta(d_tmem, ad, bd, idesc, (kb | ks | k) != 0 ? 1u : 0u);
-              else umma_bf16_2cta(d_tmem, ad, bd, idesc, (kb | ks | k) != 0 ? 1u : 0u);
-            }
-          umma_commit_2cta(&empty[stage]);
-          if (++stage == G2_STAGES) { stage = 0; phase ^= 1; }
+          const uint32_t d_tmem = tmem_base + as * G2_BN_MAX;
+          for (int kb = 0; kb < num_k; ++kb) {
+            mbar_wait(&full[stage], phase);
+            tc_fence_after();
+            const uint64_t a_desc = a_desc0 + static_cast<uint64_t>(stage) * (G2_A_STAGE >> 4);
+            const uint64_t b_desc = b_desc0 + static_cast<uint64_t>(stage) * (G2_B_STAGE >> 4);
+#pragma unroll
+            for (int ks = 0; ks < G2_KSUB; ++ks)
+#pragma unroll
+              for (int k = 0; k < BK2 / 16; ++k) {
+                const uint64_t ad = a_desc + ((ks * G2_A_BYTES + k * 32) >> 4), bd = b_desc + ((ks * G2_B_STRIDE + k * 32) >> 4);
+                if (FP8) umma_f8_2cta(d_tmem, ad, bd, idesc, (kb | ks | k) != 0 ? 1u : 0u);
+                else umma_bf16_2cta(d_tmem, ad, bd, idesc, (kb | ks | k) != 0 ? 1u : 0u);
+              }
+            umma_commit_2cta(&empty[stage]);
+            if (++stage == G2_STAGES) { stage = 0; phase ^= 1; }
+          }
+          umma_commit_2cta(&tfull[as]);
         }
-        umma_commit_2cta(&tfull[as]);
+        base += num_tiles;
       }
     }
   } else {
     const int q = warp & 3;
     int t = 0;
-    for (int tile = cluster_id; tile < num_tiles; tile += num_clusters, ++t) {
-      const int mp = tile % num_mp, n_blk = tile / num_mp;
-      const int as = t & 1;
-      const uint32_t aphase = (t >> 1) & 1;
-      mbar_wait(&tfull[as], aphase);
-      tc_fence_after();
-      const uint32_t taddr = tmem_base + (static_cast<uint32_t>(q * 32) << 16) + as * G2_BN_MAX;
-      epilogue_tile<MODE, FP8>(taddr, BN, epi_stage + (warp - 2) * (EPI_STAGE_BYTES / 4), lane,
-                               (mp * 2 + static_cast<int>(rank)) * BM2 + q * 32, n_blk * BN, M, N, ep, sa, sb);
-      tc_fence_before();
-      __syncwarp();
-      if (lane == 0) mbar_arrive_remote(&tempty[as], 0);
+    int g = cluster_id, base = 0;
+#pragma unroll
+    for (int ip = 0; ip < NPH; ++ip) {
+      const G2Phase& ph = p.ph[ip];
+      const int num_mp = (ph.M + 2 * BM2 - 1) / (2 * BM2);
+      const int num_n = (ph.N + ph.BN - 1) / ph.BN;
+      const int num_tiles = num_mp * num_n;
+      for (; g < base + num_tiles; g += num_clusters, ++t) {
+        const int tile = g - base;
+        int mp, n_blk;
+        tile_pos<NPH>(tile, num_mp, num_n, mp, n_blk);
+        const int as = t & 1;
+        const uint32_t aphase = (t >> 1) & 1;
+        mbar_wait(&tfull[as], aphase);
+        tc_fence_after();
+        const uint32_t taddr = tmem_base + (static_cast<uint32_t>(q * 32) << 16) + as * G2_BN_MAX;
+        float* st = epi_stage + (warp - 2) * (EPI_STAGE_BYTES / 4);
+        const int row0 = (mp * 2 + static_cast<int>(rank)) * BM2 + q * 32;
+        if (ip == 0) {
+          epilogue_tile<MODE0, FP8>(taddr, ph.BN, st, lane, row0, n_blk * ph.BN, ph.M, ph.N, ph.ep, p.sa, p.sb);
+        } else if constexpr (NPH == 2) {
+          epilogue_tile<MODE1, FP8>(taddr, ph.BN, st, lane, row0, n_blk * ph.BN, ph.M, ph.N, ph.ep, p.sa, p.sb);
+        }
+        tc_fence_before();
+        __syncwarp();
+        if (lane == 0) {
+          mbar_arrive_remote(&tempty[as], 0);
+          if (NPH == 2 && ip == 0) rows_publish(p.ready + mp * 2 + static_cast<int>(rank));
+        }
+      }
+      base += num_tiles;
     }
   }
   tc_fence_before();
@@ -145,30 +234,67 @@
     tc_fence_after();
     tmem_dealloc_2cta<512>(tmem_base);
   }
-}
-
-template <int MODE, bool FP8 = false>
-void launch2(const CUtensorMap& tmA, const CUtensorMap& tmB, int M, int N, int K, int BN, int a_kblock, const GemmEpi& epi,
-             cudaStream_t stream, const float* sa = nullptr, const float* sb = nullptr) {
-  auto kern = gemm_bf16_2cta<MODE, FP8>;
+  if (NPH == 2 && threadIdx.x == 0) {
+    const int row_tiles = 2 * ((p.ph[0].M + 2 * BM2 - 1) / (2 * BM2));
+    __threadfence();
+    if (atomicAdd(p.ready + GEMM_CHAIN_ROW_TILES, 1u) == gridDim.x - 1) {
+      __threadfence();
+      for (int i = 0; i < row_tiles; ++i) p.ready[i] = 0;
+      p.ready[GEMM_CHAIN_ROW_TILES] = 0;
+    }
+  }
+}
+
+G2Phase make_phase(int M, int N, int K, int bn, int a_kblock, const GemmEpi& epi) {
+  G2Phase ph;
+  ph.M = M; ph.N = N; ph.K = K; ph.BN = bn; ph.a_kblock = a_kblock; ph.ep = epi;
+  return ph;
+}
+
+int pair_tiles(const G2Phase& ph) { return ((ph.M + 2 * BM2 - 1) / (2 * BM2)) * ((ph.N + ph.BN - 1) / ph.BN); }
+
+template <int MODE0, int MODE1, bool FP8>
+void launch2(const G2Params& p, int clusters, cudaStream_t stream) {
+  auto kern = gemm_bf16_2cta<MODE0, MODE1, FP8>;
   ensure_dyn_smem(kern, G2_SMEM);
-  const int tiles = ((M + 2 * BM2 - 1) / (2 * BM2)) * ((N + BN - 1) / BN);
+  int tiles = pair_tiles(p.ph[0]);
+  if (MODE1 >= 0) tiles += pair_tiles(p.ph[1]);
+  const int grid = 2 * (tiles < clusters ? tiles : clusters);
+  launch_pdl(PDL_GEMM, kern, dim3(grid), dim3(G2_THREADS), G2_SMEM, stream, p);
+}
+
+template <bool FP8>
+void launch2_mode(const G2Params& p, cudaStream_t stream) {
   const int clusters = device_sm_count() / 2;
-  const int grid = 2 * (tiles < clusters ? tiles : clusters);
-  launch_pdl(PDL_GEMM, kern, dim3(grid), dim3(G2_THREADS), G2_SMEM, stream, tmA, tmB, M, N, K, BN, a_kblock, epi, sa, sb);
-}
-
-template <bool FP8>
-void launch2_mode(const CUtensorMap& tmA, const CUtensorMap& tmB, int M, int N, int K, int bn, int a_kblock, const GemmEpi& epi,
-                  cudaStream_t stream, const float* sa, const float* sb) {
-  switch (epi.mode) {
-    case EPI_BF16: launch2<EPI_BF16, FP8>(tmA, tmB, M, N, K, bn, a_kblock, epi, stream, sa, sb); break;
-    case EPI_GELU_BF16: launch2<EPI_GELU_BF16, FP8>(tmA, tmB, M, N, K, bn, a_kblock, epi, stream, sa, sb); break;
-    case EPI_GATE_RESID: launch2<EPI_GATE_RESID, FP8>(tmA, tmB, M, N, K, bn, a_kblock, epi, stream, sa, sb); break;
-    case EPI_F32: launch2<EPI_F32, FP8>(tmA, tmB, M, N, K, bn, a_kblock, epi, stream, sa, sb); break;
-    case EPI_SILU_BF16: launch2<EPI_SILU_BF16, FP8>(tmA, tmB, M, N, K, bn, a_kblock, epi, stream, sa, sb); break;
+  switch (p.ph[0].ep.mode) {
+    case EPI_BF16: launch2<EPI_BF16, -1, FP8>(p, clusters, stream); break;
+    case EPI_GELU_BF16: launch2<EPI_GELU_BF16, -1, FP8>(p, clusters, stream); break;
+    case EPI_GATE_RESID: launch2<EPI_GATE_RESID, -1, FP8>(p, clusters, stream); break;
+    case EPI_F32: launch2<EPI_F32, -1, FP8>(p, clusters, stream); break;
+    case EPI_SILU_BF16: launch2<EPI_SILU_BF16, -1, FP8>(p, clusters, stream); break;
     default: LTX_CHECK(false, 2, "bad GEMM epilogue mode");
   }
+}
+
+template <typename Kern>
+int chain_clusters(Kern* kern) {
+  static std::atomic<int> cached[64];
+  int dev = 0;
+  LTX_CUDA(cudaGetDevice(&dev));
+  LTX_CHECK(dev < 64, 2, "device index");
+  int n = cached[dev].load(std::memory_order_relaxed);
+  if (n == 0) {
+    ensure_dyn_smem(kern, G2_SMEM);
+    cudaLaunchConfig_t cfg = {};
+    cfg.gridDim = dim3(device_sm_count());
+    cfg.blockDim = dim3(G2_THREADS);
+    cfg.dynamicSmemBytes = G2_SMEM;
+    LTX_CUDA(cudaOccupancyMaxActiveClusters(&n, reinterpret_cast<const void*>(kern), &cfg));
+    n = n < device_sm_count() / 2 ? n : device_sm_count() / 2;
+    LTX_CHECK(n > 0, 2, "chained GEMM: no resident cluster");
+    cached[dev].store(n, std::memory_order_relaxed);
+  }
+  return n;
 }
 
 void check_tsplit(const GemmEpi& epi, int bn) {
@@ -198,15 +324,53 @@
   int bn = force_bn ? force_bn : gemm2_fit_tile_width(M, N);
   LTX_CHECK(bn >= 64 && bn <= 256 && bn % 16 == 0, 2, "2-CTA GEMM: tile width must be a multiple of 16 in [64, 256]");
   check_tsplit(epi, bn);
-  CUtensorMap tmA;
+  G2Params p = {};
   if (a_kblock > 0) {
     LTX_CHECK(a_kblock % BK2 == 0 && K % a_kblock == 0 && lda == a_kblock, 2, "GEMM: bad K-blocked A layout");
-    tmA = make_tmap_3d(A, a_kblock, M, K / a_kblock, lda, a_kblock_stride, 64, BM2);
+    p.tmA[0] = make_tmap_3d(A, a_kblock, M, K / a_kblock, lda, a_kblock_stride, 64, BM2);
   } else {
-    tmA = make_tmap_2d(A, M, K, lda, BM2);
-  }
-  CUtensorMap tmB = make_tmap_2d(B, N, K, ldb, bn / 2);
-  launch2_mode<false>(tmA, tmB, M, N, K, bn, a_kblock, epi, stream, nullptr, nullptr);
+    p.tmA[0] = make_tmap_2d(A, M, K, lda, BM2);
+  }
+  p.tmB[0] = make_tmap_2d(B, N, K, ldb, bn / 2);
+  p.ph[0] = make_phase(M, N, K, bn, a_kblock, epi);
+  launch2_mode<false>(p, stream);
+}
+
+int chain_tile_width(int M, int N0, int N1, int clusters) {
+  const int num_mp = (M + 255) / 256;
+  int best = 256;
+  double best_cost = 1e30;
+  for (int bn = 256; bn >= 64; bn -= 16) {
+    const long long tiles = static_cast<long long>(num_mp) * ((N0 + bn - 1) / bn + (N1 + bn - 1) / bn);
+    const double cost = static_cast<double>((tiles + clusters - 1) / clusters) * (bn + 100.0);
+    if (cost < best_cost - 1e-9) { best_cost = cost; best = bn; }
+  }
+  return best;
+}
+
+void launch_gemm_2cta_chain(const GemmCall& g0, const GemmCall& g1, int M, unsigned int* ready, cudaStream_t stream) {
+  LTX_CHECK(M > 0 && 2 * ((M + 2 * BM2 - 1) / (2 * BM2)) <= GEMM_CHAIN_ROW_TILES && ready != nullptr, 2,
+            "chained GEMM: too many rows, or no readiness counters");
+  LTX_CHECK(g0.epi.mode == EPI_GATE_RESID && g0.epi.resid != nullptr && g0.epi.ldr % 4 == 0 &&
+                (g0.epi.shadow == nullptr || g0.epi.lds % 4 == 0) && g1.epi.mode == EPI_BF16 && g1.epi.out != nullptr &&
+                g1.epi.ldo % 8 == 0 && g0.K == g1.K,
+            2, "chained GEMM: gate * residual (fp32, ld % 4) then bf16 (ld % 8) over the same K");
+  const int clusters = chain_clusters(gemm_bf16_2cta<EPI_GATE_RESID, EPI_BF16, false>);
+  const int bn = chain_tile_width(M, g0.N, g1.N, clusters);
+  G2Params p = {};
+  const GemmCall* g[2] = {&g0, &g1};
+  for (int i = 0; i < 2; ++i) {
+    const GemmEpi& e = g[i]->epi;
+    LTX_CHECK(g[i]->N > 0 && g[i]->K > 0 && g[i]->K % 8 == 0 && g[i]->lda % 8 == 0 && g[i]->ldb % 8 == 0, 2,
+              "GEMM: K and leading dims must be multiples of 8");
+    LTX_CHECK(e.col_block == 0 && e.tsplit_col == 0 && e.transpose_out == 0 && e.ws == nullptr, 2,
+              "chained GEMM: row-major epilogues only");
+    p.tmA[i] = make_tmap_2d(g[i]->A, M, g[i]->K, g[i]->lda, BM2);
+    p.tmB[i] = make_tmap_2d(g[i]->B, g[i]->N, g[i]->K, g[i]->ldb, bn / 2);
+    p.ph[i] = make_phase(M, g[i]->N, g[i]->K, bn, 0, e);
+  }
+  p.ready = ready;
+  launch2<EPI_GATE_RESID, EPI_BF16, false>(p, clusters, stream);
 }
 
 void launch_gemm_fp8(const uint8_t* A, int64_t lda, const float* sa, const uint8_t* B, int64_t ldb, const float* sb, int M, int N,
@@ -227,9 +391,12 @@
   const int bn = force_bn ? force_bn : gemm2_fit_tile_width(M, N);
   LTX_CHECK(bn >= 64 && bn <= 256 && bn % 16 == 0, 2, "2-CTA GEMM: tile width must be a multiple of 16 in [64, 256]");
   check_tsplit(epi, bn);
-  const CUtensorMap tmA = make_tmap_u8_sw128(A, M, K, lda, BM2);
-  const CUtensorMap tmB = make_tmap_u8_sw128(B, N, K, ldb, bn / 2);
-  launch2_mode<true>(tmA, tmB, M, N, K, bn, 0, epi, stream, sa, sb);
-}
-
-}
+  G2Params p = {};
+  p.tmA[0] = make_tmap_u8_sw128(A, M, K, lda, BM2);
+  p.tmB[0] = make_tmap_u8_sw128(B, N, K, ldb, bn / 2);
+  p.ph[0] = make_phase(M, N, K, bn, 0, epi);
+  p.sa = sa; p.sb = sb;
+  launch2_mode<true>(p, stream);
+}
+
+}
diff --git a/ltx-video-swift-mlx_b200/csrc/ltx_internal.h b/ltx-video-swift-mlx_b200/csrc/ltx_internal.h
--- a/ltx-video-swift-mlx_b200/csrc/ltx_internal.h
+++ b/ltx-video-swift-mlx_b200/csrc/ltx_internal.h
@@ -116,6 +116,16 @@
 void launch_gemm_2cta(const bf16* A, int64_t lda, const bf16* B, int64_t ldb, int M, int N, int K, const GemmEpi& epi,
                       cudaStream_t stream, int force_bn, int a_kblock, int64_t a_kblock_stride);
 int gemm2_fit_tile_width(int M, int N);
+struct GemmCall {
+  const bf16* A = nullptr;
+  int64_t lda = 0;
+  const bf16* B = nullptr;
+  int64_t ldb = 0;
+  int N = 0, K = 0;
+  GemmEpi epi;
+};
+constexpr int GEMM_CHAIN_ROW_TILES = 4096;
+void launch_gemm_2cta_chain(const GemmCall& g0, const GemmCall& g1, int M, unsigned int* ready, cudaStream_t stream);
 void launch_gemm_fp8(const uint8_t* A, int64_t lda, const float* sa, const uint8_t* B, int64_t ldb, const float* sb, int M, int N,
                      int K, const GemmEpi& epi, cudaStream_t stream, int force_bn = 0);
 void launch_quantize_rows_fp8(const bf16* x, int64_t ld, int M, int K, uint8_t* q, float* s, cudaStream_t stream);
```

Result: slower. 25.45 (median of 6 runs) (-2.1%).
